# Senryoku/zflac

Hardware: AMD Instinct MI355X
Metric: Msamples/s decoded (bit-exact) + achieved HBM GB/s, 4096-blk stereo (higher is better)
Workload: dtype int32; 1 GPU; C5 shard: 1250 stereo 16-bit mid/side FLAC streams/GPU x 32 frames x 4096 samples, LPC order 8, partition order 4; streams_total=1250, parallelism=stream-shard x1

## Files before the change

### include/zflac_hip.h

```cpp
#ifndef ZFLAC_HIP_H
#define ZFLAC_HIP_H

#include <stddef.h>
#include <stdint.h>

#ifdef __cplusplus
extern "C" {
#endif

#define ZFLAC_OK 0
#define ZFLAC_E_INVALID_SIGNATURE 1
#define ZFLAC_E_INVALID_METADATA_HEADER 2
#define ZFLAC_E_MISSING_STREAMINFO 3
#define ZFLAC_E_UNIMPLEMENTED 4
#define ZFLAC_E_INVALID_CHECKSUM 5
#define ZFLAC_E_INVALID_FRAME_HEADER 6
#define ZFLAC_E_INCONSISTENT_PARAMETERS 7
#define ZFLAC_E_INVALID_CODED_NUMBER 8
#define ZFLAC_E_INVALID_SUBFRAME_HEADER 9
#define ZFLAC_E_INVALID_RESIDUAL_CODING 10
#define ZFLAC_E_END_OF_STREAM 11
#define ZFLAC_E_OUT_OF_MEMORY 12
#define ZFLAC_E_DEVICE 13
#define ZFLAC_E_INVALID_ARGUMENT 14
#define ZFLAC_E_OUT_OF_DOMAIN 15
#define ZFLAC_E_FRAME_CRC 16

#define ZFLAC_S8 0
#define ZFLAC_S16 1
#define ZFLAC_S32 2

typedef struct zflac_info {
    uint8_t channels;
    uint8_t bits_per_sample;
    uint8_t sample_kind;
    uint8_t reserved;
    uint32_t sample_rate;
    uint64_t n_samples;
    uint64_t samples_bytes;
} zflac_info;

typedef struct zflac_stream {
    const uint8_t *data;
    size_t len;
} zflac_stream;

typedef struct zflac_timings {
    double scan_ms;
    double decode_ms;
    double verify_ms;
    double total_ms;
    uint64_t frames;
    uint64_t input_bytes;
    uint64_t output_bytes;
    uint64_t samples;
    double walk_ms;
    double md5_ms;
    double plan_ms;
    double upload_ms;
    double run_wall_ms;
    double read_ms;
    double host_md5_ms;
    double crc16_ms;
    uint32_t rest_launches;
    uint32_t sequential_streams;
} zflac_timings;

typedef struct zflac_batch zflac_batch;

int zflac_hip_open(const uint8_t *buf, size_t len, int device, zflac_batch **out_batch, zflac_info *info);
int zflac_hip_open_ex(const uint8_t *buf, size_t len, int device, int flags, zflac_batch **out_batch,
                      zflac_info *info);
int zflac_hip_read(zflac_batch *b, void *out_samples, size_t out_bytes);
void zflac_hip_close(zflac_batch *b);

int zflac_hip_batch_create(const zflac_stream *streams, size_t n, int device, int flags, zflac_batch **out);
int zflac_hip_batch_run(zflac_batch *b);
int zflac_hip_batch_submit(zflac_batch *b);
int zflac_hip_batch_wait(zflac_batch *b);
int zflac_hip_batch_ready(zflac_batch *b);
int zflac_hip_batch_info(zflac_batch *b, size_t i, zflac_info *info);
int zflac_hip_batch_read(zflac_batch *b, size_t i, void *out, size_t out_bytes, int verify_md5);
int zflac_hip_batch_md5(zflac_batch *b, size_t i, uint8_t *digest16);
const void *zflac_hip_batch_device_samples(zflac_batch *b, size_t i);
int zflac_hip_batch_timings(zflac_batch *b, zflac_timings *t);
int zflac_hip_batch_timings_ex(zflac_batch *b, zflac_timings *t, size_t size);
#define ZFLAC_TIMINGS_V1_SIZE 80
#define ZFLAC_BUCKET_8 1u
#define ZFLAC_BUCKET_4 2u
#define ZFLAC_BUCKET_16 4u
#define ZFLAC_BUCKET_32 8u
#define ZFLAC_BUCKET_MIX_8 16u
#define ZFLAC_BUCKET_MIX_32 32u
#define ZFLAC_BUCKET_12 64u
#define ZFLAC_BUCKET_ALL 127u
int zflac_hip_batch_decode_buckets(zflac_batch *b, uint32_t *used, uint32_t *planned);
size_t zflac_hip_batch_size(zflac_batch *b);
void zflac_hip_batch_destroy(zflac_batch *b);

#define ZFLAC_EXPORT_F32 0
#define ZFLAC_EXPORT_F16 1
#define ZFLAC_EXPORT_BF16 2
#define ZFLAC_EXPORT_I32 3
#define ZFLAC_LAYOUT_PLANAR 0
#define ZFLAC_LAYOUT_INTERLEAVED 1
typedef struct zflac_export_desc {
    uint32_t size;
    uint8_t dtype, layout;
    uint16_t channels;
    uint64_t frames;
    const uint64_t *starts;
} zflac_export_desc;
int zflac_hip_batch_export(zflac_batch *b, const zflac_export_desc *d, void *dst_device, size_t dst_bytes,
                           uint64_t *valid_frames, void *stream);
int zflac_hip_batch_export_ms(zflac_batch *b, double *ms);

typedef struct zflac_resample_desc {
    uint32_t size;
    uint8_t dtype, layout;
    uint16_t channels;
    uint64_t frames;
    const uint64_t *starts;
    uint32_t sample_rate;
    uint16_t zeros;
    uint16_t reserved;
    double rolloff;
    double beta;
} zflac_resample_desc;
int zflac_hip_batch_export_resampled(zflac_batch *b, const zflac_resample_desc *d, void *dst_device,
                                     size_t dst_bytes, uint64_t *valid_frames, void *stream);
uint64_t zflac_hip_resampled_frames(uint64_t n_frames, uint32_t rate_in, uint32_t rate_out);
int zflac_hip_batch_resample_tables(zflac_batch *b, uint64_t *built, uint64_t *held_floats);

#define ZFLAC_FLAG_TIMING 1
#define ZFLAC_FLAG_FORCE_SLOW 2
#define ZFLAC_FLAG_DEVICE_MD5 4
#define ZFLAC_FLAG_CHECK_CRC16 8
#define ZFLAC_FLAG_WALK_LANE 16
#define ZFLAC_FLAG_WALK_WAVE 32

const char *zflac_hip_error_name(int code);
int zflac_hip_device_count(void);
const char *zflac_hip_version(void);
const char *zflac_hip_build_id(void);
#define ZFLAC_HIP_ABI_VERSION 5
int zflac_hip_abi_version(void);

#ifdef __cplusplus
}
#endif
#endif
```

### zflac_amd/_lib.py

```python
from __future__ import annotations

import ctypes
import os

_HERE = os.path.dirname(os.path.abspath(__file__))
lib_path = os.environ.get("ZFLAC_HIP_LIB") or os.path.join(_HERE, "libzflac_hip.so")


class zflac_info(ctypes.Structure):
    _fields_ = [("channels", ctypes.c_uint8), ("bits_per_sample", ctypes.c_uint8),
                ("sample_kind", ctypes.c_uint8), ("reserved", ctypes.c_uint8),
                ("sample_rate", ctypes.c_uint32), ("n_samples", ctypes.c_uint64),
                ("samples_bytes", ctypes.c_uint64)]


class zflac_stream(ctypes.Structure):
    _fields_ = [("data", ctypes.c_void_p), ("len", ctypes.c_size_t)]


class zflac_timings(ctypes.Structure):
    _fields_ = [("scan_ms", ctypes.c_double), ("decode_ms", ctypes.c_double), ("verify_ms", ctypes.c_double),
                ("total_ms", ctypes.c_double), ("frames", ctypes.c_uint64), ("input_bytes", ctypes.c_uint64),
                ("output_bytes", ctypes.c_uint64), ("samples", ctypes.c_uint64), ("walk_ms", ctypes.c_double),
                ("md5_ms", ctypes.c_double), ("plan_ms", ctypes.c_double), ("upload_ms", ctypes.c_double),
                ("run_wall_ms", ctypes.c_double), ("read_ms", ctypes.c_double), ("host_md5_ms", ctypes.c_double),
                ("crc16_ms", ctypes.c_double), ("rest_launches", ctypes.c_uint32), ("sequential_streams", ctypes.c_uint32)]


class zflac_export_desc(ctypes.Structure):
    _fields_ = [("size", ctypes.c_uint32), ("dtype", ctypes.c_uint8), ("layout", ctypes.c_uint8),
                ("channels", ctypes.c_uint16), ("frames", ctypes.c_uint64), ("starts", ctypes.POINTER(ctypes.c_uint64))]


class zflac_resample_desc(ctypes.Structure):
    _fields_ = [("size", ctypes.c_uint32), ("dtype", ctypes.c_uint8), ("layout", ctypes.c_uint8),
                ("channels", ctypes.c_uint16), ("frames", ctypes.c_uint64), ("starts", ctypes.POINTER(ctypes.c_uint64)),
                ("sample_rate", ctypes.c_uint32), ("zeros", ctypes.c_uint16), ("reserved", ctypes.c_uint16),
                ("rolloff", ctypes.c_double), ("beta", ctypes.c_double)]


_P = ctypes.c_void_p
SIGNATURES = {
    "zflac_hip_open": (ctypes.c_int, [ctypes.c_char_p, ctypes.c_size_t, ctypes.c_int, ctypes.POINTER(_P),
                                      ctypes.POINTER(zflac_info)]),
    "zflac_hip_open_ex": (ctypes.c_int, [ctypes.c_char_p, ctypes.c_size_t, ctypes.c_int, ctypes.c_int,
                                         ctypes.POINTER(_P), ctypes.POINTER(zflac_info)]),
    "zflac_hip_read": (ctypes.c_int, [_P, _P, ctypes.c_size_t]),
    "zflac_hip_close": (None, [_P]),
    "zflac_hip_batch_create": (ctypes.c_int, [ctypes.POINTER(zflac_stream), ctypes.c_size_t, ctypes.c_int,
                                              ctypes.c_int, ctypes.POINTER(_P)]),
    "zflac_hip_batch_run": (ctypes.c_int, [_P]),
    "zflac_hip_batch_submit": (ctypes.c_int, [_P]),
    "zflac_hip_batch_wait": (ctypes.c_int, [_P]),
    "zflac_hip_batch_ready": (ctypes.c_int, [_P]),
    "zflac_hip_batch_info": (ctypes.c_int, [_P, ctypes.c_size_t, ctypes.POINTER(zflac_info)]),
    "zflac_hip_batch_read": (ctypes.c_int, [_P, ctypes.c_size_t, _P, ctypes.c_size_t, ctypes.c_int]),
    "zflac_hip_batch_md5": (ctypes.c_int, [_P, ctypes.c_size_t, ctypes.c_char_p]),
    "zflac_hip_batch_device_samples": (_P, [_P, ctypes.c_size_t]),
    "zflac_hip_batch_timings": (ctypes.c_int, [_P, ctypes.POINTER(zflac_timings)]),
    "zflac_hip_batch_timings_ex": (ctypes.c_int, [_P, ctypes.POINTER(zflac_timings), ctypes.c_size_t]),
    "zflac_hip_abi_version": (ctypes.c_int, []),
    "zflac_hip_batch_export": (ctypes.c_int, [_P, ctypes.POINTER(zflac_export_desc), _P, ctypes.c_size_t,
                                              ctypes.POINTER(ctypes.c_uint64), _P]),
    "zflac_hip_batch_export_ms": (ctypes.c_int, [_P, ctypes.POINTER(ctypes.c_double)]),
    "zflac_hip_batch_export_resampled": (ctypes.c_int, [_P, ctypes.POINTER(zflac_resample_desc), _P, ctypes.c_size_t,
                                                        ctypes.POINTER(ctypes.c_uint64), _P]),
    "zflac_hip_resampled_frames": (ctypes.c_uint64, [ctypes.c_uint64, ctypes.c_uint32, ctypes.c_uint32]),
    "zflac_hip_batch_resample_tables": (ctypes.c_int, [_P, ctypes.POINTER(ctypes.c_uint64),
                                                       ctypes.POINTER(ctypes.c_uint64)]),
    "zflac_hip_batch_decode_buckets": (ctypes.c_int, [_P, ctypes.POINTER(ctypes.c_uint32),
                                                      ctypes.POINTER(ctypes.c_uint32)]),
    "zflac_hip_batch_size": (ctypes.c_size_t, [_P]),
    "zflac_hip_batch_destroy": (None, [_P]),
    "zflac_hip_error_name": (ctypes.c_char_p, [ctypes.c_int]),
    "zflac_hip_device_count": (ctypes.c_int, []),
    "zflac_hip_version": (ctypes.c_char_p, []),
    "zflac_hip_build_id": (ctypes.c_char_p, []),
}

FLAG_TIMING = 1
FLAG_FORCE_SLOW = 2
FLAG_DEVICE_MD5 = 4
FLAG_CHECK_CRC16 = 8
FLAG_WALK_LANE = 16
FLAG_WALK_WAVE = 32
EXPORT_F32 = 0
EXPORT_F16 = 1
EXPORT_BF16 = 2
EXPORT_I32 = 3
LAYOUT_PLANAR = 0
LAYOUT_INTERLEAVED = 1
BUCKET_8 = 1
BUCKET_4 = 2
BUCKET_16 = 4
BUCKET_32 = 8
BUCKET_MIX_8 = 16
BUCKET_MIX_32 = 32
BUCKET_12 = 64
BUCKET_ALL = 127

_lib = None


def load():
    global _lib
    if _lib is None:
        if not os.path.exists(lib_path):
            try:
                from . import build as _build

                _build.build()
            except Exception as e:
                raise RuntimeError(f"libzflac_hip.so is missing and could not be built: {e}") from e
        lib = ctypes.CDLL(lib_path)
        for name, (res, args) in SIGNATURES.items():
            fn = getattr(lib, name)
            fn.restype = res
            fn.argtypes = args
        _lib = lib
    return _lib
```

### zflac_amd/api.py

```python
from __future__ import annotations

import ctypes
import dataclasses

import numpy as np

from . import _lib, errors

_DTYPES = {0: np.int8, 1: np.int16, 2: np.int32}
_TAGS = {0: "s8", 1: "s16", 2: "s32"}


@dataclasses.dataclass
class Samples:

    tag: str
    values: np.ndarray

    @property
    def s8(self) -> np.ndarray:
        return self._arm("s8")

    @property
    def s16(self) -> np.ndarray:
        return self._arm("s16")

    @property
    def s32(self) -> np.ndarray:
        return self._arm("s32")

    def _arm(self, tag):
        if self.tag != tag:
            raise AttributeError(f"inactive union field {tag!r} (active: {self.tag!r})")
        return self.values


@dataclasses.dataclass
class DecodedFLAC:

    channels: int
    sample_rate: int
    bits_per_sample: int
    samples: Samples

    def deinit(self, allocator=None) -> None:
        self.samples = Samples(self.samples.tag, self.samples.values[:0])


def _read_all(reader) -> bytes:
    if isinstance(reader, (bytes, bytearray, memoryview)):
        return bytes(reader)
    if hasattr(reader, "read"):
        return reader.read()
    raise TypeError("decode() expects bytes or a reader with .read()")


def device_count() -> int:
    return _lib.load().zflac_hip_device_count()


def build_id() -> str:
    return _lib.load().zflac_hip_build_id().decode()


def _aligned_empty(nbytes: int, dtype) -> np.ndarray:
    raw = np.empty(nbytes + 32, dtype=np.uint8)
    off = (-raw.ctypes.data) % 32
    return raw[off:off + nbytes].view(dtype)


def decode(reader, device: int = 0, timings: dict | None = None, check_crc16: bool = False) -> DecodedFLAC:
    data = _read_all(reader)
    L = _lib.load()
    handle = ctypes.c_void_p()
    info = _lib.zflac_info()
    flags = _lib.FLAG_CHECK_CRC16 if check_crc16 else 0
    rc = L.zflac_hip_open_ex(data, len(data), device, flags, ctypes.byref(handle), ctypes.byref(info))
    try:
        errors.check(rc)
        out = _aligned_empty(info.samples_bytes, _DTYPES[info.sample_kind])
        rc = L.zflac_hip_read(handle, out.ctypes.data_as(ctypes.c_void_p) if info.samples_bytes else None,
                              info.samples_bytes)
        errors.check(rc)
        if timings is not None:
            t = _lib.zflac_timings()
            L.zflac_hip_batch_timings_ex(handle, ctypes.byref(t), ctypes.sizeof(t))
            timings.update({name: getattr(t, name) for name, _ in _lib.zflac_timings._fields_})
        return DecodedFLAC(info.channels, info.sample_rate, info.bits_per_sample,
                           Samples(_TAGS[info.sample_kind], out))
    finally:
        if handle:
            L.zflac_hip_close(handle)


class Batch:

    def __init__(self, streams, device: int = 0, timing: bool = False, force_slow: bool = False,
                 device_md5: bool = False, check_crc16: bool = False, walk: str | None = None):
        self._L = _lib.load()
        self.device = device
        self._bufs = [bytes(s) for s in streams]
        arr = (_lib.zflac_stream * len(self._bufs))()
        self._keep = []
        for i, b in enumerate(self._bufs):
            cb = ctypes.create_string_buffer(b, len(b))
            self._keep.append(cb)
            arr[i].data = ctypes.cast(cb, ctypes.c_void_p)
            arr[i].len = len(b)
        flags = ((_lib.FLAG_TIMING if timing else 0) | (_lib.FLAG_FORCE_SLOW if force_slow else 0)
                 | (_lib.FLAG_DEVICE_MD5 if device_md5 else 0) | (_lib.FLAG_CHECK_CRC16 if check_crc16 else 0)
                 | {None: 0, "lane": _lib.FLAG_WALK_LANE, "wave": _lib.FLAG_WALK_WAVE}[walk])
        self._h = ctypes.c_void_p()
        rc = self._L.zflac_hip_batch_create(arr, len(self._bufs), device, flags, ctypes.byref(self._h))
        self._keep = None
        errors.check(rc, "batch_create")

    def __len__(self):
        return len(self._bufs)

    def run(self) -> None:
        errors.check(self._L.zflac_hip_batch_run(self._h), "batch_run")

    def submit(self) -> None:
        errors.check(self._L.zflac_hip_batch_submit(self._h), "batch_submit")

    def wait(self) -> None:
        errors.check(self._L.zflac_hip_batch_wait(self._h), "batch_wait")

    def ready(self) -> bool:
        rc = self._L.zflac_hip_batch_ready(self._h)
        if rc < 0:
            errors.check(-rc, "batch_ready")
        return rc == 1

    def info(self, i: int):
        inf = _lib.zflac_info()
        rc = self._L.zflac_hip_batch_info(self._h, i, ctypes.byref(inf))
        return rc, inf

    def error_name(self, i: int) -> str:
        return errors.NAMES.get(self.info(i)[0], "Unknown")

    def read(self, i: int, verify_md5: bool = True) -> DecodedFLAC:
        rc, inf = self.info(i)
        errors.check(rc)
        out = _aligned_empty(inf.samples_bytes, _DTYPES[inf.sample_kind])
        rc = self._L.zflac_hip_batch_read(self._h, i, out.ctypes.data_as(ctypes.c_void_p) if inf.samples_bytes
                                          else None, inf.samples_bytes, 1 if verify_md5 else 0)
        errors.check(rc)
        return DecodedFLAC(inf.channels, inf.sample_rate, inf.bits_per_sample, Samples(_TAGS[inf.sample_kind], out))

    def md5(self, i: int):
        buf = ctypes.create_string_buffer(16)
        rc = self._L.zflac_hip_batch_md5(self._h, i, buf)
        return None if rc else buf.raw

    def timings(self):
        t = _lib.zflac_timings()
        rc = self._L.zflac_hip_batch_timings_ex(self._h, ctypes.byref(t), ctypes.sizeof(t))
        return None if rc else t

    def decode_buckets(self):
        used, planned = ctypes.c_uint32(), ctypes.c_uint32()
        errors.check(self._L.zflac_hip_batch_decode_buckets(self._h, ctypes.byref(used), ctypes.byref(planned)),
                     "batch_decode_buckets")
        return used.value, planned.value

    def device_samples(self, i: int) -> int:
        return self._L.zflac_hip_batch_device_samples(self._h, i) or 0

    def close(self):
        if getattr(self, "_h", None):
            self._L.zflac_hip_batch_destroy(self._h)
            self._h = None

    def __del__(self):
        try:
            self.close()
        except Exception:
            pass


def decode_many(streams, device: int = 0, verify_md5: bool = True, device_md5: bool = True):
    b = Batch(streams, device, device_md5=device_md5 and verify_md5)
    try:
        b.run()
        out = []
        for i in range(len(b)):
            try:
                out.append(b.read(i, verify_md5))
            except errors.ZflacError as e:
                out.append(e)
        return out
    finally:
        b.close()
```

### zflac_amd/build.py

```python
from __future__ import annotations

import os
import subprocess
import sys
import time

HERE = os.path.dirname(os.path.abspath(__file__))
ROOT = os.path.dirname(HERE)
CSRC = os.path.join(HERE, "csrc")
LIB = os.path.join(HERE, "libzflac_hip.so")
SOURCES = [os.path.join(CSRC, f"decode_k{k}_{lay}{mix}.hip") for k in (1, 2, 0) for lay in ("stereo", "mono", "multi")
           for mix in ("", "_mix")]
SOURCES += [os.path.join(CSRC, n) for n in ("scan.hip", "md5.hip", "crc16.hip", "walk_wave.hip", "export.hip",
                                            "resample.hip", "stream_plan.cpp", "resample_plan.cpp", "pipeline.cpp",
                                            "seq_planner.cpp", "md5_host.cpp", "abi.cpp")]
HEADERS = [os.path.join(CSRC, n) for n in ("common.h", "frame_header.h", "device_common.h", "launch.h", "stream_plan.h",
                                           "resample_plan.h", "export_tile.h", "batch.h", "md5.hpp", "decode.inc")]
DEPS = SOURCES + HEADERS + [os.path.join(ROOT, "include", "zflac_hip.h")]
ARCH = os.environ.get("ZFLAC_OFFLOAD_ARCH", "gfx950")
CFLAGS = ["-O3", "-std=c++20", "-fPIC", "-Wall", "-Wno-unused-function"]


def source_fingerprint(defines=()) -> str:
    import hashlib

    h = hashlib.sha256(f"{ARCH}|{' '.join(CFLAGS)}|{' '.join(sorted(defines))}".encode())
    for d in sorted(DEPS):
        h.update(os.path.basename(d).encode())
        with open(d, "rb") as f:
            h.update(f.read())
    return h.hexdigest()


def sources_present() -> bool:
    return all(os.path.exists(d) for d in DEPS)


def needs_build() -> bool:
    if not os.path.exists(LIB):
        return True
    t = os.path.getmtime(LIB)
    return any(os.path.getmtime(d) > t for d in DEPS)


def lib_build_id(path: str | None = None) -> str | None:
    import re

    try:
        with open(path or LIB, "rb") as f:
            m = re.search(rb"src=([0-9a-f]{64})", f.read())
    except OSError:
        return None
    return m.group(0).decode() if m else None


def _obj_deps(src: str):
    if src.endswith("abi.cpp"):
        return list(DEPS)
    hdrs = [h for h in HEADERS if not h.endswith("decode.inc") or "decode_k" in src]
    return [src] + hdrs + [os.path.join(ROOT, "include", "zflac_hip.h")]


def build(force: bool = False, verbose: bool = False, defines=(), out: str | None = None, units=None) -> str:
    lib = out or LIB
    if not force and not defines and not out and not needs_build():
        return LIB
    if units:
        build()
        units = set(units) | {"abi.cpp"}
    objs = []
    tag = "_".join(d.replace("=", "-") for d in defines)
    build_dir = os.path.join(HERE, "_build" + ("_" + tag if tag else ""))
    os.makedirs(build_dir, exist_ok=True)
    procs = []
    fp = source_fingerprint(defines)
    jobs = max(1, min(int(os.environ.get("MAX_JOBS", "8")), os.cpu_count() or 1, 16))
    for src in SOURCES:
        if units and os.path.basename(src) not in units:
            objs.append(os.path.join(HERE, "_build", os.path.basename(src) + ".o"))
            continue
        obj = os.path.join(build_dir, os.path.basename(src) + ".o")
        if not force and os.path.exists(obj) and os.path.getmtime(obj) >= max(os.path.getmtime(d)
                                                                               for d in _obj_deps(src)):
            objs.append(obj)
            continue
        cmd = ["hipcc", f"--offload-arch={ARCH}"] + CFLAGS + ["-I", os.path.join(ROOT, "include"), "-c", src, "-o", obj]
        cmd[1:1] = [f"-D{d}" for d in defines]
        if src.endswith(".hip"):
            cmd[1:1] = ["-x", "hip"]
        if src.endswith("_plan.cpp"):
            cmd[1:1] = ["-x", "c++"]
        if src.endswith("abi.cpp"):
            cmd[1:1] = [f'-DZFLAC_BUILD_ID="src={fp}"']
        if verbose:
            print(" ".join(cmd))
        while sum(p.poll() is None for _, p in procs) >= jobs:
            time.sleep(0.2)
        procs.append((src, subprocess.Popen(cmd)))
        objs.append(obj)
    failed = [src for src, p in procs if p.wait() != 0]
    if failed:
        raise RuntimeError(f"hipcc failed for {failed}")
    os.makedirs(os.path.dirname(lib), exist_ok=True)
    cmd = ["hipcc", f"--offload-arch={ARCH}", "-shared", "-fPIC", "-o", lib] + objs
    subprocess.check_call(cmd)
    return lib


if __name__ == "__main__":
    a = sys.argv[1:]
    out = a[a.index("-o") + 1] if "-o" in a else None
    units = a[a.index("--units") + 1].split(",") if "--units" in a else None
    build(force="--force" in a, verbose=True, defines=[x[2:] for x in a if x.startswith("-D")], out=out, units=units)
```

### zflac_amd/csrc/abi.cpp

```cpp
#include <cstring>
#include <new>
#include <vector>

#include "batch.h"
#include "launch.h"

using namespace zflac;

zflac_batch::~zflac_batch() {
    if (exp_pending) (void)hipEventSynchronize(ev_exp);
    if (stream) (void)hipStreamSynchronize(stream);
    if (ev_done) (void)hipEventSynchronize(ev_done);
    if (md5_pending) {
        try {
            hub_release(this);
        } catch (...) {
        }
        try {
            hub_forget(this);
        } catch (...) {
        }
    }
    if (md5_hub && ev_md5) (void)hipEventSynchronize(ev_md5);
    if (front) (void)hipStreamSynchronize(front);
    classes.clear();
    for (auto& s : streams) s.override_out.reset();
    for (auto& e : ev)
        if (e) (void)hipEventDestroy(e);
    if (ev_done) (void)hipEventDestroy(ev_done);
    if (ev_md5) (void)hipEventDestroy(ev_md5);
    if (pipe_pin) (void)hipHostFree(pipe_pin);
    if (exp_pin) (void)hipHostFree(exp_pin);
    if (ev_exp_copy) (void)hipEventDestroy(ev_exp_copy);
    if (ev_exp) (void)hipEventDestroy(ev_exp);
    for (auto& e : ev_exp_t)
        if (e) (void)hipEventDestroy(e);
    if (stream) (void)hipStreamDestroy(stream);
    if (front) (void)hipStreamDestroy(front);
    if (front_join) (void)hipEventDestroy(front_join);
}

namespace {

struct ExportShape {
    size_t n;
    uint64_t T, C, esz, tiles;
    uint32_t vec;
};

bool export_shape(zflac_batch* b, uint32_t size, uint32_t want_size, int dtype, int max_dtype, int layout,
                  uint64_t channels, uint64_t frames, const void* dst, size_t dst_bytes, ExportShape& s) {
    if (!b || !dst || size != want_size) return false;
    if (dtype > max_dtype || layout > ZFLAC_LAYOUT_INTERLEAVED || !channels || !frames) return false;
    if (!b->ran || b->submitted) return false;
    s.n = b->streams.size();
    s.T = frames;
    s.C = channels;
    s.esz = (dtype == ZFLAC_EXPORT_F16 || dtype == ZFLAC_EXPORT_BF16) ? 2 : 4;
    const unsigned __int128 need = (unsigned __int128)s.n * s.C * s.T * s.esz;
    if (need > (unsigned __int128)dst_bytes) return false;
    s.tiles = (s.T + EXPORT_TILE - 1) / EXPORT_TILE;
    if ((unsigned __int128)s.n * s.tiles > 0x7FFFFFFFull) return false;
    const uint64_t row_bytes = (layout == ZFLAC_LAYOUT_PLANAR ? s.T : s.T * s.C) * s.esz;
    s.vec = (reinterpret_cast<uintptr_t>(dst) % 16 == 0 && row_bytes % 16 == 0) ? 1u : 0u;
    return true;
}

ExportRow export_row(const StreamState& s, uint64_t start) {
    ExportRow r;
    std::memset(&r, 0, sizeof(r));
    r.start = start;
    r.kind = s.info.sample_kind;
    if (!s.err && s.info.channels && s.dev_samples) {
        r.nch = s.info.channels;
        r.n_frames = s.info.n_samples / s.info.channels;
        if (r.start < r.n_frames) r.src = s.dev_samples;
    }
    return r;
}

bool export_begin(zflac_batch* b, size_t n, void* stream, hipStream_t st) {
    if (!b->exp_pin) {
        ck(hipHostMalloc(reinterpret_cast<void**>(&b->exp_pin), n * sizeof(ResampleRow), hipHostMallocDefault));
        b->exp_rows.alloc(n * sizeof(ResampleRow));
        ck(hipEventCreateWithFlags(&b->ev_exp_copy, hipEventDisableTiming));
        ck(hipEventCreateWithFlags(&b->ev_exp, hipEventDisableTiming));
    }
    if (b->exp_any) {
        ck(hipEventSynchronize(b->ev_exp_copy));
        ck(hipStreamWaitEvent(st, b->ev_exp, 0));
    }
    const bool timed = !stream && (b->flags & ZFLAC_FLAG_TIMING);
    if (timed)
        for (auto& e : b->ev_exp_t)
            if (!e) ck(hipEventCreate(&e));
    return timed;
}

template <typename Launch>
void export_run(zflac_batch* b, size_t bytes, bool timed, void* stream, hipStream_t st, Launch launch) {
    if (timed) ck(hipEventRecord(b->ev_exp_t[0], st));
    ck(hipMemcpyAsync(b->exp_rows.p, b->exp_pin, bytes, hipMemcpyHostToDevice, st));
    ck(hipEventRecord(b->ev_exp_copy, st));
    const hipError_t le = launch();
    ck(hipEventRecord(b->ev_exp, st));
    b->exp_any = true;
    ck(le);
    if (timed) ck(hipEventRecord(b->ev_exp_t[1], st));
    if (stream) {
        b->exp_pending = true;
    } else {
        ck(hipStreamSynchronize(st));
        if (timed) {
            float ms = 0;
            ck(hipEventElapsedTime(&ms, b->ev_exp_t[0], b->ev_exp_t[1]));
            b->export_ms = ms;
        }
    }
}

ResampleTable* resample_table(zflac_batch* b, uint32_t fin, const zflac_resample_desc* d, const ResampleRatio& ratio) {
    for (auto& t : b->rs_tables)
        if (t->fin == fin && t->fout == d->sample_rate && t->zeros == d->zeros && t->rolloff == d->rolloff &&
            t->beta == d->beta)
            return t.get();
    auto t = std::make_unique<ResampleTable>();
    t->fin = fin;
    t->fout = d->sample_rate;
    t->zeros = d->zeros;
    t->rolloff = d->rolloff;
    t->beta = d->beta;
    t->ratio = ratio;
    std::vector<float> h;
    resample_taps(ratio, d->zeros, d->beta, h);
    t->taps.alloc(h.size());
    ck(hipMemcpy(t->taps.p, h.data(), h.size() * sizeof(float), hipMemcpyHostToDevice));
    b->rs_built++;
    b->rs_tables.push_back(std::move(t));
    return b->rs_tables.back().get();
}

}

extern "C" {

const char* zflac_hip_error_name(int code) {
    switch (code) {
        case 0: return "OK";
        case 1: return "InvalidSignature";
        case 2: return "InvalidMetadataHeader";
        case 3: return "MissingStreaminfo";
        case 4: return "Unimplemented";
        case 5: return "InvalidChecksum";
        case 6: return "InvalidFrameHeader";
        case 7: return "InconsistentParameters";
        case 8: return "InvalidCodedNumber";
        case 9: return "InvalidSubframeHeader";
        case 10: return "InvalidResidualCodingMethod";
        case 11: return "EndOfStream";
        case 12: return "OutOfMemory";
        case 13: return "DeviceError";
        case 14: return "InvalidArgument";
        case 15: return "OutOfDomain";
        case 16: return "FrameCrcMismatch";
        default: return "Unknown";
    }
}

int zflac_hip_device_count(void) {
    int n = 0;
    if (hipGetDeviceCount(&n) != hipSuccess) return 0;
    return n;
}

const char* zflac_hip_version(void) { return "zflac_hip gfx950 r4"; }

#ifndef ZFLAC_BUILD_ID
#define ZFLAC_BUILD_ID "unknown"
#endif
const char* zflac_hip_build_id(void) { return ZFLAC_BUILD_ID; }

int zflac_hip_batch_create(const zflac_stream* streams, size_t n, int device, int flags, zflac_batch** out) {
    return create_batch(streams, n, device, flags, out);
}

static void drain_failed_submit(zflac_batch* b) {
    try {
        hub_forget(b);
    } catch (...) {
    }
    (void)hipStreamSynchronize(b->stream);
    if (b->rs) (void)hipStreamSynchronize(b->rs);
    if (b->front) (void)hipStreamSynchronize(b->front);
    b->rs = b->stream;
    b->submitted = false;
}

int zflac_hip_batch_submit(zflac_batch* b) {
    if (!b || b->submitted) return E_INVALID_ARGUMENT;
    b->ran = false;
    try {
        b->submit_t0 = now_ms();
        b->submitted = true;
        submit_batch(b);
    } catch (const DeviceError&) {
        drain_failed_submit(b);
        return E_DEVICE;
    } catch (const std::bad_alloc&) {
        drain_failed_submit(b);
        return E_OUT_OF_MEMORY;
    } catch (const std::exception&) {
        drain_failed_submit(b);
        return E_DEVICE;
    }
    return E_OK;
}

int zflac_hip_batch_wait(zflac_batch* b) {
    if (!b || !b->submitted) return E_INVALID_ARGUMENT;
    b->submitted = false;
    int rc = E_OK;
    try {
        finish_batch(b);
        b->timings.run_wall_ms = now_ms() - b->submit_t0;
        b->ran = true;
    } catch (const DeviceError&) {
        rc = E_DEVICE;
    } catch (const std::bad_alloc&) {
        rc = E_OUT_OF_MEMORY;
    } catch (const std::exception&) {
        rc = E_DEVICE;
    }
    if (rc != E_OK && b->md5_pending) {
        try {
            hub_forget(b);
        } catch (...) {
        }
    }
    return rc;
}

int zflac_hip_batch_ready(zflac_batch* b) {
    if (!b || !b->submitted) return -E_INVALID_ARGUMENT;
    hipError_t e = hipEventQuery(b->ev_done);
    if (e == hipSuccess && b->md5_hub) {
        try {
            Md5Hub& h = md5_hub(b->device);
            std::lock_guard<std::mutex> lock(h.mu);
            if (b->md5_pending) {
                if (!h.any || hipEventQuery(h.last) == hipSuccess) hub_flush(h);
                return 0;
            }
            if (b->md5_failed) return -E_DEVICE;
        } catch (const DeviceError&) {
            return -E_DEVICE;
        }
        e = hipEventQuery(b->ev_md5);
    }
    if (e == hipSuccess) return 1;
    if (e == hipErrorNotReady) return 0;
    return -E_DEVICE;
}

int zflac_hip_batch_run(zflac_batch* b) {
    const int rc = zflac_hip_batch_submit(b);
    return rc ? rc : zflac_hip_batch_wait(b);
}

size_t zflac_hip_batch_size(zflac_batch* b) { return b ? b->streams.size() : 0; }

int zflac_hip_batch_info(zflac_batch* b, size_t i, zflac_info* info) {
    if (!b || !b->ran || i >= b->streams.size()) return E_INVALID_ARGUMENT;
    const StreamState& s = b->streams[i];
    if (info) *info = s.info;
    return s.err;
}

const void* zflac_hip_batch_device_samples(zflac_batch* b, size_t i) {
    if (!b || !b->ran || i >= b->streams.size() || b->streams[i].err) return nullptr;
    return b->streams[i].dev_samples;
}

int zflac_hip_batch_read(zflac_batch* b, size_t i, void* out, size_t out_bytes, int verify_md5) {
    if (!b || !b->ran || i >= b->streams.size()) return E_INVALID_ARGUMENT;
    StreamState& s = b->streams[i];
    if (s.err) return s.err;
    if (out_bytes < s.info.samples_bytes || (!out && s.info.samples_bytes)) return E_INVALID_ARGUMENT;
    try {
        ck(hipSetDevice(b->device));
        return read_samples(b, s, out, verify_md5 && !s.md5_dev);
    } catch (const DeviceError&) {
        return E_DEVICE;
    } catch (const std::exception&) {
        return E_DEVICE;
    }
}

int zflac_hip_batch_md5(zflac_batch* b, size_t i, uint8_t* digest) {
    if (!b || !b->ran || i >= b->streams.size() || !digest) return E_INVALID_ARGUMENT;
    const StreamState& s = b->streams[i];
    if (!s.md5_dev) return E_INVALID_ARGUMENT;
    std::memcpy(digest, s.md5_dig, 16);
    return E_OK;
}

int zflac_hip_batch_timings(zflac_batch* b, zflac_timings* t) {
    return zflac_hip_batch_timings_ex(b, t, ZFLAC_TIMINGS_V1_SIZE);
}

int zflac_hip_batch_timings_ex(zflac_batch* b, zflac_timings* t, size_t size) {
    if (!b || !t || size == 0) return E_INVALID_ARGUMENT;
    std::memcpy(t, &b->timings, std::min(size, sizeof(zflac_timings)));
    if (size > sizeof(zflac_timings)) std::memset(reinterpret_cast<uint8_t*>(t) + sizeof(zflac_timings), 0,
                                                  size - sizeof(zflac_timings));
    return b->have_timing ? E_OK : E_INVALID_ARGUMENT;
}

int zflac_hip_abi_version(void) { return ZFLAC_HIP_ABI_VERSION; }

int zflac_hip_batch_export(zflac_batch* b, const zflac_export_desc* d, void* dst_device, size_t dst_bytes,
                           uint64_t* valid_frames, void* stream) {
    ExportShape s;
    if (!d || !export_shape(b, d->size, sizeof(zflac_export_desc), d->dtype, ZFLAC_EXPORT_I32, d->layout, d->channels,
                            d->frames, dst_device, dst_bytes, s))
        return E_INVALID_ARGUMENT;
    const size_t n = s.n;
    for (size_t i = 0; valid_frames && i < n; i++) {
        const StreamState& st = b->streams[i];
        const uint64_t start = d->starts ? d->starts[i] : 0;
        const uint64_t nf = (st.err || !st.info.channels) ? 0 : st.info.n_samples / st.info.channels;
        valid_frames[i] = nf > start ? std::min(nf - start, s.T) : 0;
    }
    if (n == 0) return E_OK;
    try {
        DeviceScope scope(b->device);
        hipStream_t st = stream ? static_cast<hipStream_t>(stream) : b->stream;
        const bool timed = export_begin(b, n, stream, st);
        ExportRow* rows = reinterpret_cast<ExportRow*>(b->exp_pin);
        for (size_t i = 0; i < n; i++) rows[i] = export_row(b->streams[i], d->starts ? d->starts[i] : 0);
        ExportArgs a;
        std::memset(&a, 0, sizeof(a));
        a.rows = reinterpret_cast<const ExportRow*>(b->exp_rows.p);
        a.dst = dst_device;
        a.frames = s.T;
        a.channels = (uint32_t)s.C;
        a.n_rows = (uint32_t)n;
        a.tiles = (uint32_t)s.tiles;
        a.vec = s.vec;
        export_run(b, n * sizeof(ExportRow), timed, stream, st,
                   [&] { return launch_export(d->dtype, d->layout, a, st); });
    } catch (const DeviceError&) {
        return E_DEVICE;
    } catch (const std::bad_alloc&) {
        return E_OUT_OF_MEMORY;
    }
    return E_OK;
}

uint64_t zflac_hip_resampled_frames(uint64_t n_frames, uint32_t rate_in, uint32_t rate_out) {
    return resampled_frames(n_frames, rate_in, rate_out);
}

int zflac_hip_batch_export_resampled(zflac_batch* b, const zflac_resample_desc* d, void* dst_device, size_t dst_bytes,
                                     uint64_t* valid_frames, void* stream) {
    ExportShape s;
    if (!d || !export_shape(b, d->size, sizeof(zflac_resample_desc), d->dtype, ZFLAC_EXPORT_BF16, d->layout,
                            d->channels, d->frames, dst_device, dst_bytes, s))
        return E_INVALID_ARGUMENT;
    if (!d->sample_rate || d->sample_rate > RESAMPLE_MAX_RATE || d->reserved ||
        !resample_params_ok(d->zeros, d->rolloff, d->beta))
        return E_INVALID_ARGUMENT;
    const size_t n = s.n;
    struct Need {
        uint32_t fin;
        ResampleRatio ratio;
    };
    std::vector<Need> needs;
    std::vector<int> plan(n, -1);
    std::vector<uint64_t> n_out(n, 0);
    uint64_t floats = 0, tiles = s.tiles;
    try {
        for (size_t i = 0; i < n; i++) {
            const StreamState& st = b->streams[i];
            if (st.err || !st.info.channels || !st.info.sample_rate) continue;
            const uint64_t nf = st.info.n_samples / st.info.channels;
            const uint32_t fin = st.info.sample_rate;
            if (fin == d->sample_rate) {
                n_out[i] = nf;
                continue;
            }
            n_out[i] = resampled_frames(nf, fin, d->sample_rate);
            int k = 0;
            while (k < (int)needs.size() && needs[k].fin != fin) k++;
            if (k == (int)needs.size()) {
                Need nd;
                nd.fin = fin;
                if (!resample_ratio(fin, d->sample_rate, d->zeros, d->rolloff, nd.ratio)) return E_INVALID_ARGUMENT;
                if (nd.ratio.K > RESAMPLE_MAX_TAPS) return E_INVALID_ARGUMENT;
                floats += nd.ratio.table_floats();
                if (floats > RESAMPLE_MAX_TABLE_FLOATS) return E_INVALID_ARGUMENT;
                needs.push_back(nd);
            }
            plan[i] = k;
            const ResampleTile rt = resample_tile(needs[k].ratio, std::min<uint64_t>(st.info.channels, s.C));
            tiles = std::max(tiles, (s.T + rt.tile - 1) / rt.tile);
        }
    } catch (const std::bad_alloc&) {
        return E_OUT_OF_MEMORY;
    }
    if ((unsigned __int128)n * tiles > 0x7FFFFFFFull) return E_INVALID_ARGUMENT;
    for (size_t i = 0; valid_frames && i < n; i++) {
        const uint64_t start = d->starts ? d->starts[i] : 0;
        valid_frames[i] = n_out[i] > start ? std::min(n_out[i] - start, s.T) : 0;
    }
    if (n == 0) return E_OK;
    try {
        DeviceScope scope(b->device);
        hipStream_t st = stream ? static_cast<hipStream_t>(stream) : b->stream;
        uint64_t held = 0;
        for (auto& t : b->rs_tables) held += t->ratio.table_floats();
        if (held + floats > RESAMPLE_MAX_TABLE_FLOATS) {
            std::erase_if(b->rs_tables, [&](const std::unique_ptr<ResampleTable>& t) {
                if (t->fout == d->sample_rate && t->zeros == d->zeros && t->rolloff == d->rolloff && t->beta == d->beta)
                    for (const Need& nd : needs)
                        if (nd.fin == t->fin) return false;
                return true;
            });
        }
        std::vector<const ResampleTable*> tabs;
        for (const Need& nd : needs) tabs.push_back(resample_table(b, nd.fin, d, nd.ratio));
        const bool timed = export_begin(b, n, stream, st);
        ResampleRow* rows = reinterpret_cast<ResampleRow*>(b->exp_pin);
        for (size_t i = 0; i < n; i++) {
            const StreamState& ss = b->streams[i];
            ResampleRow r;
            std::memset(&r, 0, sizeof(r));
            const uint64_t start = d->starts ? d->starts[i] : 0;
            if (plan[i] < 0) {
                r.e = export_row(ss, start);
                if (!n_out[i]) r.e.src = nullptr;
            } else {
                const ResampleTable* t = tabs[plan[i]];
                const ResampleTile rt = resample_tile(t->ratio, std::min<uint64_t>(ss.info.channels, s.C));
                r.e = export_row(ss, 0);
                r.e.start = start;
                r.n_out = n_out[i];
                if (r.e.src && start < r.n_out) {
                    r.taps = t->taps.p;
                    r.L = t->ratio.L;
                    r.M = t->ratio.M;
                    r.W = t->ratio.W;
                    r.K = (uint32_t)t->ratio.K;
                    r.tile = rt.tile;
                    r.cg = rt.cg;
                    r.tab_lds = rt.tab_lds;
                } else {
                    r.e.src = nullptr;
                }
            }
            rows[i] = r;
        }
        ResampleArgs a;
        std::memset(&a, 0, sizeof(a));
        a.rows = reinterpret_cast<const ResampleRow*>(b->exp_rows.p);
        a.dst = dst_device;
        a.frames = s.T;
        a.channels = (uint32_t)s.C;
        a.n_rows = (uint32_t)n;
        a.tiles = (uint32_t)tiles;
        a.vec = s.vec;
        export_run(b, n * sizeof(ResampleRow), timed, stream, st,
                   [&] { return launch_resample(d->dtype, d->layout, a, st); });
    } catch (const DeviceError&) {
        return E_DEVICE;
    } catch (const std::bad_alloc&) {
        return E_OUT_OF_MEMORY;
    }
    return E_OK;
}

int zflac_hip_batch_resample_tables(zflac_batch* b, uint64_t* built, uint64_t* held_floats) {
    if (!b) return E_INVALID_ARGUMENT;
    if (built) *built = b->rs_built;
    if (held_floats) {
        *held_floats = 0;
        for (auto& t : b->rs_tables) *held_floats += t->ratio.table_floats();
    }
    return E_OK;
}

static_assert(ZFLAC_BUCKET_8 == bucket_bit(8, false) && ZFLAC_BUCKET_4 == bucket_bit(4, false) &&
                  ZFLAC_BUCKET_16 == bucket_bit(16, false) && ZFLAC_BUCKET_32 == bucket_bit(32, false) &&
                  ZFLAC_BUCKET_MIX_8 == bucket_bit(8, true) && ZFLAC_BUCKET_MIX_32 == bucket_bit(32, true) &&
                  ZFLAC_BUCKET_12 == bucket_bit(12, false) && ZFLAC_BUCKET_ALL == BUCKET_MASK_ALL,
              "ZFLAC_BUCKET_* (zflac_hip.h) and bucket_bit() (common.h) disagree");

int zflac_hip_batch_decode_buckets(zflac_batch* b, uint32_t* used, uint32_t* planned) {
    if (!b || !used || !planned || !b->ran || b->submitted) return E_INVALID_ARGUMENT;
    *used = b->buckets_used;
    *planned = b->buckets_planned;
    return E_OK;
}

int zflac_hip_batch_export_ms(zflac_batch* b, double* ms) {
    if (!b || !ms || b->export_ms < 0) return E_INVALID_ARGUMENT;
    *ms = b->export_ms;
    return E_OK;
}

#ifdef ZFLAC_PROBE
extern "C" int zflac_hip_probe(zflac_batch* b, unsigned long long* out, int n) {
    if (!b || b->classes.empty() || n > (int)(PROBE_BYTES / 8)) return E_INVALID_ARGUMENT;
    auto& C = *b->classes[0];
    uint8_t* p = reinterpret_cast<uint8_t*>(C.dummy.p) + DUMMY_BYTES;
    if (hipMemcpy(out, p, n * 8, hipMemcpyDeviceToHost) != hipSuccess) return E_DEVICE;
    if (hipMemset(p, 0, PROBE_BYTES) != hipSuccess) return E_DEVICE;
    return E_OK;
}
#endif

#ifdef ZFLAC_REPLAY
extern "C" int zflac_hip_replay(zflac_batch** bs, int nb, int reps, int what, double* ms) {
    try {
        if (nb <= 0 || !bs || !ms) return E_INVALID_ARGUMENT;
        ck(hipSetDevice(bs[0]->device));
        for (int i = 0; i < nb; i++) {
            ck(hipStreamSynchronize(bs[i]->rs));
            bs[i]->rs = next_run_stream(bs[i]->device);
        }
        const double t0 = now_ms();
        for (int r = 0; r < reps; r++) {
            for (int i = 0; i < nb; i++) {
                zflac_batch* b = bs[i];
                Class& C = *b->classes[0];
                if (what == 4) {
                    enqueue_class(b, C, false, false);
                    continue;
                }
                if (what >= 8) {
                    const ScanArgs sa = scan_args(C);
                    ck(launch_scan(sa, b->rs));
                    if (what == 16) {
                        ck(launch_scan_chunks(C.chunk_cnt.p, C.chunk_units.p, sa.n_chunks, C.chunk_off.p,
                                              C.chunk_uoff.p, C.misc.p, b->rs));
                        ck(launch_compact(compact_args(C), b->rs));
                    }
                    continue;
                }
                DecodeArgs da = decode_args(C);
                da.full_mask = C.full_mask;
                const uint32_t mf = std::min(C.grid_frames, C.cap);
                if (what & 1) ck(launch_walk_k1(da, mf, b->rs));
                if (what & 2) ck(launch_decode_k1_stereo(da, mf, b->rs));
            }
        }
        for (int i = 0; i < nb; i++) ck(hipStreamSynchronize(bs[i]->rs));
        *ms = now_ms() - t0;
        for (int i = 0; i < nb; i++) bs[i]->rs = bs[i]->stream;
        return E_OK;
    } catch (const DeviceError&) {
        return E_DEVICE;
    }
}
#endif

void zflac_hip_batch_destroy(zflac_batch* b) {
    if (!b) return;
    (void)hipSetDevice(b->device);
    delete b;
}

int zflac_hip_open(const uint8_t* buf, size_t len, int device, zflac_batch** out_batch, zflac_info* info) {
    return zflac_hip_open_ex(buf, len, device, 0, out_batch, info);
}

int zflac_hip_open_ex(const uint8_t* buf, size_t len, int device, int flags, zflac_batch** out_batch,
                      zflac_info* info) {
    if (!out_batch) return E_INVALID_ARGUMENT;
    zflac_stream s{buf, len};
    int rc = create_batch(&s, 1, device, flags, out_batch);
    if (rc) return rc;
    rc = zflac_hip_batch_run(*out_batch);
    if (rc) return rc;
    return zflac_hip_batch_info(*out_batch, 0, info);
}

int zflac_hip_read(zflac_batch* b, void* out_samples, size_t out_bytes) {
    return zflac_hip_batch_read(b, 0, out_samples, out_bytes, 1);
}

void zflac_hip_close(zflac_batch* b) { zflac_hip_batch_destroy(b); }

}
```

### zflac_amd/csrc/batch.h

```cpp
#pragma once
#include <hip/hip_runtime.h>

#include <algorithm>
#include <atomic>
#include <chrono>
#include <cstdint>
#include <memory>
#include <mutex>
#include <vector>

#include "../../include/zflac_hip.h"
#include "common.h"
#include "resample_plan.h"
#include "stream_plan.h"

namespace zflac {

inline double now_ms() {
    return std::chrono::duration<double, std::milli>(std::chrono::steady_clock::now().time_since_epoch()).count();
}

struct DeviceError {};
inline void ck(hipError_t e) {
    if (e != hipSuccess) throw DeviceError{};
}

template <typename T>
struct DevBuf {
    T* p = nullptr;
    size_t n = 0;
    DevBuf() = default;
    DevBuf(const DevBuf&) = delete;
    DevBuf& operator=(const DevBuf&) = delete;
    ~DevBuf() { release(); }
    void release() {
        if (p) (void)hipFree(p);
        p = nullptr;
        n = 0;
    }
    void alloc(size_t count) {
        if (count <= n && p) return;
        release();
        ck(hipMalloc(reinterpret_cast<void**>(&p), std::max<size_t>(count, 1) * sizeof(T)));
        n = count;
    }
};

struct ResampleTable {
    uint32_t fin = 0, fout = 0, zeros = 0;
    double rolloff = 0, beta = 0;
    ResampleRatio ratio;
    DevBuf<float> taps;
};

struct StreamState : StreamPlan {
    int cls = -1;
    uint32_t slot = 0;
    int err = 0;
    zflac_info info = {};
    const void* dev_samples = nullptr;
    int md5_dev = 0;
    uint8_t md5_dig[16] = {};
    std::unique_ptr<DevBuf<uint8_t>> override_out;
};

struct Class {
    int kind = 1;
    int nch = 2;
    std::vector<uint32_t> members;
    std::vector<StreamDesc> desc;
    std::vector<ChunkDesc> chunks;
    uint64_t in_bytes = 0, out_elems = 0;
    uint32_t cap = 0;
    uint64_t est_frames = 0;
    uint32_t grid_frames = 0;
    uint32_t full_mask = 0;
    bool redone = false;
    DevBuf<uint8_t> in;
    DevBuf<uint8_t> out;
    DevBuf<StreamDesc> d_desc;
    DevBuf<ChunkDesc> d_chunks;
    DevBuf<uint32_t> chunk_cnt, chunk_off, chunk_slot_units, misc;
    uint32_t* status = nullptr;
    DevBuf<unsigned long long> chunk_units, chunk_uoff;
    DevBuf<uint64_t> chunk_slots;
    DevBuf<uint64_t> c_pos, c_out, c_end;
    DevBuf<uint32_t> c_stream, c_info, c_rate, sub, group_mb;
    DevBuf<int32_t> c_err;
    DevBuf<uint32_t> crc_bad;
    DevBuf<uint8_t> dummy;
    struct Pinned {
        uint32_t* p = nullptr;
        ~Pinned() {
            if (p) (void)hipHostFree(p);
        }
    } pin;
    uint32_t* h_misc = nullptr;
    uint32_t* h_status = nullptr;
    bool any_unknown = false;
    DevBuf<uint64_t> units;
    uint64_t* h_units = nullptr;
};

struct DeviceScope {
    int prev = -1;
    explicit DeviceScope(int dev) {
        if (hipGetDevice(&prev) != hipSuccess) prev = -1;
        if (prev != dev) ck(hipSetDevice(dev));
    }
    ~DeviceScope() {
        int cur = -1;
        if (prev >= 0 && hipGetDevice(&cur) == hipSuccess && cur != prev) (void)hipSetDevice(prev);
    }
};

struct Uploader {
    static constexpr uint64_t WIN = 32ull << 20;
    std::mutex mu;
    uint8_t* pin[2] = {nullptr, nullptr};
    hipEvent_t done[2] = {nullptr, nullptr};
    bool used[2] = {false, false};
};

constexpr int MAX_HUB_STREAMS = 4;
struct Md5Hub {
    std::mutex mu;
    hipStream_t st[MAX_HUB_STREAMS] = {};
    uint32_t n_st = 1, next = 0;
    hipEvent_t last = nullptr;
    bool any = false;
    std::vector<zflac_batch*> pend;
    uint32_t runs = 8;
    int device = 0;
};

constexpr int MAX_RUN_STREAMS = 8;
struct DeviceStreams {
    std::mutex mu;
    hipStream_t run[MAX_RUN_STREAMS] = {};
    uint32_t n_run = 3, next = 0;
    Md5Hub hub;
    DeviceStreams();
};

DeviceStreams& device_streams(int device);
Md5Hub& md5_hub(int device);
hipStream_t next_run_stream(int device);
void hub_flush(Md5Hub& h);
void hub_release(zflac_batch* b);
void hub_forget(zflac_batch* b);
int read_samples(zflac_batch* b, StreamState& s, void* out, bool hash);
void plan_md5_pipeline(zflac_batch* b);
void finish_md5(zflac_batch* b, bool timing);

DecodeArgs decode_args(Class& C);
ScanArgs scan_args(Class& C);
CompactArgs compact_args(Class& C);
hipError_t launch_decode(int kind, const DecodeArgs& a, uint32_t max_frames, hipStream_t st,
                         hipEvent_t mid = nullptr, hipStream_t front = nullptr, hipEvent_t join = nullptr,
                         uint64_t est_frames = 0, int flags = 0);
void enqueue_class(zflac_batch* b, Class& C, bool timing_first, bool timing_last);
void submit_batch(zflac_batch* b);
void finish_batch(zflac_batch* b);
int create_batch(const zflac_stream* streams, size_t n, int device, int flags, zflac_batch** out);

void finish_stream_sequential(zflac_batch* b, Class& C, uint32_t slot, const std::vector<uint32_t>& h_chunk_off,
                              uint32_t nframes);

}

struct zflac_batch {
    int device = 0;
    int flags = 0;
    hipStream_t stream = nullptr;
    hipStream_t front = nullptr;
    hipEvent_t front_join = nullptr;
    std::vector<zflac::StreamState> streams;
    std::vector<std::unique_ptr<zflac::Class>> classes;
    hipEvent_t ev[10] = {};
    hipEvent_t ev_done = nullptr;
    hipStream_t rs = nullptr;
    hipEvent_t ev_md5 = nullptr;
    std::atomic<bool> md5_pending{false};
    bool md5_failed = false;
    bool md5_hub = false;
    bool have_timing = false;
    bool ran = false;
    bool submitted = false;
    double submit_t0 = 0;
    zflac::DevBuf<zflac::Md5Job> md5_jobs;
    zflac::DevBuf<uint32_t> md5_dig;
    zflac::DevBuf<zflac::Md5Job> pipe_jobs;
    int pipe_coop = -1;
    zflac::DevBuf<uint32_t> pipe_dig;
    std::vector<uint32_t> pipe_who;
    uint32_t* pipe_pin = nullptr;
    zflac_timings timings = {};
    uint8_t* exp_pin = nullptr;
    zflac::DevBuf<uint8_t> exp_rows;
    hipEvent_t ev_exp_copy = nullptr, ev_exp = nullptr;
    hipEvent_t ev_exp_t[2] = {};
    bool exp_any = false;
    bool exp_pending = false;
    double export_ms = -1;
    std::vector<std::unique_ptr<zflac::ResampleTable>> rs_tables;
    uint64_t rs_built = 0;
    uint32_t buckets_used = 0, buckets_planned = 0;
    ~zflac_batch();
};
```

### zflac_amd/csrc/common.h

```cpp
#pragma once
#include <cstdint>

#ifdef __HIPCC__
#define ZFLAC_HD __host__ __device__
#else
#define ZFLAC_HD
#endif

namespace zflac {

enum Err : int {
    E_OK = 0,
    E_INVALID_SIGNATURE = 1,
    E_INVALID_METADATA_HEADER = 2,
    E_MISSING_STREAMINFO = 3,
    E_UNIMPLEMENTED = 4,
    E_INVALID_CHECKSUM = 5,
    E_INVALID_FRAME_HEADER = 6,
    E_INCONSISTENT_PARAMETERS = 7,
    E_INVALID_CODED_NUMBER = 8,
    E_INVALID_SUBFRAME_HEADER = 9,
    E_INVALID_RESIDUAL_CODING = 10,
    E_END_OF_STREAM = 11,
    E_OUT_OF_MEMORY = 12,
    E_DEVICE = 13,
    E_INVALID_ARGUMENT = 14,
    E_OUT_OF_DOMAIN = 15,
    E_FRAME_CRC = 16,
};

struct StreamDesc {
    uint64_t in_begin;
    uint64_t in_end;
    uint64_t out_base;
    uint64_t out_cap;
    uint64_t total;
    uint32_t rate_hz;
    uint32_t si_rate;
    uint32_t first_chunk;
    uint32_t end_chunk;
    uint8_t byte1;
    uint8_t nch;
    uint8_t dcode;
    uint8_t si_bps;
    uint8_t valid_total;
    uint8_t justify;
    uint8_t pad_[2];
};

struct ChunkDesc {
    uint64_t begin;
    uint64_t end;
    uint32_t stream;
    uint32_t pad_;
};

constexpr uint32_t INFO_PRE_ERR = 1u << 28;
constexpr uint32_t INFO_CRC_EOF = 1u << 29;

constexpr int SCAN_THREADS = 256;
#ifndef ZFLAC_SCAN_BPT
#define ZFLAC_SCAN_BPT 128
#endif
constexpr int SCAN_BYTES_PER_THREAD = ZFLAC_SCAN_BPT;
constexpr uint64_t CHUNK_BYTES = (uint64_t)SCAN_THREADS * SCAN_BYTES_PER_THREAD;
constexpr int CHUNK_CAP = 64;
constexpr uint64_t INPUT_PAD = 4096;
constexpr int MAX_CH = 8;
#ifndef ZFLAC_WAVE_WALK_MAX_FRAMES
#define ZFLAC_WAVE_WALK_MAX_FRAMES 16384
#endif
constexpr uint64_t WAVE_WALK_MAX_FRAMES = ZFLAC_WAVE_WALK_MAX_FRAMES;
constexpr uint64_t DUMMY_BYTES = 64 * 64 * 32;
constexpr uint64_t PROBE_BYTES = 256;

struct ScanArgs {
    const uint8_t* in;
    const StreamDesc* streams;
    const ChunkDesc* chunks;
    uint32_t n_chunks;
    uint32_t* chunk_cnt;
    unsigned long long* chunk_units;
    uint64_t* chunk_slots;
    uint32_t* chunk_slot_units;
    uint32_t* status;
    uint32_t n_status;
    uint32_t* misc;
};

struct CompactArgs {
    const uint8_t* in;
    const StreamDesc* streams;
    const ChunkDesc* chunks;
    uint32_t n_chunks;
    const uint32_t* chunk_cnt;
    const uint64_t* chunk_slots;
    const uint32_t* chunk_slot_units;
    const uint32_t* chunk_off;
    const unsigned long long* chunk_uoff;
    uint32_t cap;
    uint64_t* c_pos;
    uint32_t* c_stream;
    uint64_t* c_out;
    uint32_t* overflow;
};

struct DecodeArgs {
    const uint8_t* in;
    uint64_t in_size;
    void* out;
    const StreamDesc* streams;
    const uint64_t* c_pos;
    const uint32_t* c_stream;
    const uint64_t* c_out;
    const uint32_t* n_frames;
    uint32_t n_frames_host;
    uint32_t cap;
    uint64_t* c_end;
    int32_t* c_err;
    uint32_t* c_info;
    uint32_t* c_rate;
    int nch;
    int write;
    void* dummy;
    uint32_t* sub_start;
    uint32_t* group_mb;
    uint32_t* bucket_used;
    uint32_t full_mask;
    uint32_t rest;
    uint32_t rest_only;
};

constexpr uint32_t SPARSE_DECODE_BLOCKS = 256;

ZFLAC_HD inline constexpr uint32_t bucket_bit(uint32_t mb, bool mix) {
    return mix ? (mb <= 8 ? 16u : 32u)
               : (mb == 8 ? 1u : (mb == 4 ? 2u : (mb == 16 ? 4u : (mb == 12 ? 64u : 8u))));
}
constexpr uint32_t BUCKET_MASK_ALL = 127u;

enum Md5Mode : uint32_t {
    MD5_RAW = 0,
    MD5_S16_SHIFT = 1,
    MD5_S32_SHIFT = 2,
    MD5_S24 = 3,
};

struct Md5Job {
    const uint8_t* data;
    uint64_t n;
    uint32_t mode;
    uint32_t js;
    uint32_t width;
    uint32_t pad_;
    const uint32_t* status;
};

constexpr int MD5_MAX_SEGS = 16;
struct Md5Segs {
    const Md5Job* jobs[MD5_MAX_SEGS];
    uint32_t* dig[MD5_MAX_SEGS];
    uint32_t start[MD5_MAX_SEGS + 1];
    uint32_t nseg;
};

struct VerifyArgs {
    const StreamDesc* streams;
    uint32_t n_streams;
    const uint32_t* chunk_off;
    const uint64_t* c_pos;
    const uint32_t* c_stream;
    const uint64_t* c_out;
    const uint32_t* n_frames;
    uint32_t cap;
    const uint64_t* c_end;
    const int32_t* c_err;
    const uint32_t* c_info;
    const uint32_t* c_rate;
    uint32_t* status;
    uint64_t* units;
};

struct SyncListArgs {
    const uint8_t* in;
    uint64_t lo, hi;
    uint64_t in_end;
    uint32_t si_rate;
    uint32_t rate_hz;
    uint32_t nch, dcode;
    uint64_t* pos;
    uint32_t* count;
    uint32_t cap;
};

struct Crc16Args {
    const uint8_t* in;
    uint64_t in_size;
    const uint64_t* pos;
    const uint64_t* end;
    const int32_t* err;
    const StreamDesc* streams;
    const uint32_t* c_stream;
    const uint64_t* c_out;
    const uint32_t* n_frames;
    uint32_t n_frames_host;
    uint32_t cap;
    uint32_t* bad;
};

struct ExportRow {
    const void* src;
    uint64_t n_frames;
    uint64_t start;
    uint8_t nch;
    uint8_t kind;
    uint8_t pad_[6];
};
static_assert(sizeof(ExportRow) == 32, "ExportRow is the 32-byte record host and kernel share");

constexpr uint32_t EXPORT_THREADS = 256;
constexpr uint32_t EXPORT_GROUP = 16;
constexpr uint64_t EXPORT_TILE = (uint64_t)EXPORT_THREADS * EXPORT_GROUP;

struct ExportArgs {
    const ExportRow* rows;
    void* dst;
    uint64_t frames;
    uint32_t channels;
    uint32_t n_rows;
    uint32_t tiles;
    uint32_t vec;
};

struct ResampleRow {
    ExportRow e;
    const float* taps;
    uint64_t n_out;
    uint32_t L, M;
    uint32_t W, K;
    uint32_t tile;
    uint8_t cg;
    uint8_t tab_lds;
    uint8_t pad_[2];
};
static_assert(sizeof(ResampleRow) == 72, "ResampleRow is the 72-byte record host and kernel share");

constexpr uint32_t RESAMPLE_THREADS = 512;
constexpr uint32_t RESAMPLE_LDS_FLOATS = 20480;
constexpr uint32_t RESAMPLE_LDS_TABLE = 16896;
constexpr uint32_t RESAMPLE_MAX_TILE = 2048;
constexpr uint32_t RESAMPLE_MAX_CG = 4;

struct ResampleArgs {
    const ResampleRow* rows;
    void* dst;
    uint64_t frames;
    uint32_t channels;
    uint32_t n_rows;
    uint32_t tiles;
    uint32_t vec;
};

}
```

### zflac_amd/csrc/device_common.h

```cpp
#pragma once
#include <hip/hip_runtime.h>

#include <atomic>
#include <cstdint>
#include <utility>

#include "common.h"
#include "frame_header.h"

namespace zflac {

__device__ __forceinline__ uint32_t bswap32(uint32_t x) { return __builtin_bswap32(x); }

static __constant__ Crc8Table CRC8 = make_crc8_table();

__device__ __forceinline__ FrameHdr parse_frame_header(const uint8_t* p, uint64_t avail, uint32_t si_rate) {
    return parse_frame_header_t<1>([p](uint32_t i) -> uint32_t { return p[i]; }, avail, si_rate, CRC8.t);
}
__device__ __forceinline__ FrameHdr parse_frame_fields(const uint8_t* p, uint64_t avail, uint32_t si_rate) {
    return parse_frame_header_t<0>([p](uint32_t i) -> uint32_t { return p[i]; }, avail, si_rate, nullptr);
}

__device__ __forceinline__ bool candidate_ok(const FrameHdr& h, const StreamDesc& S) {
    return h.err == 0 && !h.crc_eof && h.crc_ok && h.zero_bit == 0 && h.byte1 == S.byte1 &&
           channels_count(h.chan_code) == S.nch && h.dcode == S.dcode && h.rate == S.rate_hz;
}

}
```

### zflac_amd/csrc/frame_header.h

```cpp
#pragma once
#include <cstdint>

#include "common.h"

#define ZFLAC_HDI ZFLAC_HD inline __attribute__((always_inline))
#ifdef __clang__
#define ZFLAC_UNROLL _Pragma("unroll")
#else
#define ZFLAC_UNROLL _Pragma("GCC unroll 8")
#endif

namespace zflac {

ZFLAC_HDI int channels_count(uint32_t code) {
    return code <= 7 ? (int)code + 1 : (code <= 10 ? 2 : 0);
}
ZFLAC_HDI uint32_t rate_table(uint32_t code) {
    switch (code) {
        case 1: return 88200;
        case 2: return 176400;
        case 3: return 192000;
        case 4: return 8000;
        case 5: return 16000;
        case 6: return 22050;
        case 7: return 24000;
        case 8: return 32000;
        case 9: return 44100;
        case 10: return 48000;
        default: return 96000;
    }
}
ZFLAC_HDI int depth_bits(uint32_t dcode, int si_bps) {
    switch (dcode) {
        case 0: return si_bps;
        case 1: return 8;
        case 2: return 12;
        case 4: return 16;
        case 5: return 20;
        case 6: return 24;
        case 7: return 32;
        default: return -1;
    }
}

struct Crc8Table {
    uint8_t t[256];
};
constexpr Crc8Table make_crc8_table() {
    Crc8Table r{};
    for (int i = 0; i < 256; i++) {
        uint32_t c = (uint32_t)i;
        for (int k = 0; k < 8; k++) c = (c & 0x80) ? ((c << 1) ^ 0x07) & 0xFF : (c << 1) & 0xFF;
        r.t[i] = (uint8_t)c;
    }
    return r;
}

constexpr uint32_t crc8_reduce(uint32_t a) {
    for (int i = 0; i < 4; i++) {
        const uint32_t t = a >> 8;
        a = (t ^ (t << 1) ^ (t << 2)) ^ (a & 0xFFu);
    }
    return a;
}
constexpr uint32_t crc8_3(uint32_t crc, uint32_t w) { return crc8_reduce((w ^ (crc << 16)) << 8); }
constexpr uint32_t crc8_1(uint32_t crc, uint32_t b) { return crc8_reduce((crc ^ b) << 8); }
constexpr bool crc8_fold_matches_table() {
    const Crc8Table t = make_crc8_table();
    for (uint32_t i = 0; i < 256; i++)
        if (crc8_1(0, i) != t.t[i]) return false;
    uint32_t a = 0, b = 0, x = 12345;
    for (int k = 0; k < 300; k++) {
        uint32_t w = 0;
        for (int j = 0; j < 3; j++) {
            x = x * 1103515245u + 12345u;
            const uint32_t by = (x >> 16) & 0xFFu;
            a = t.t[a ^ by];
            w = (w << 8) | by;
        }
        b = crc8_3(b, w);
        if (a != b) return false;
    }
    return true;
}
static_assert(crc8_fold_matches_table(), "register CRC-8 = table CRC-8");

struct FrameHdr {
    uint32_t bs, rate, hdr_len;
    uint32_t chan_code, dcode, byte1, zero_bit, bs_code;
    int err;
    bool crc_eof;
    bool crc_ok;
};

template <int CRC, typename At>
ZFLAC_HDI FrameHdr parse_frame_header_t(At&& at, uint64_t avail, uint32_t si_rate, const uint8_t* crc_tab) {
    FrameHdr h;
    h.bs = h.rate = h.hdr_len = 0;
    h.chan_code = h.dcode = h.byte1 = h.zero_bit = h.bs_code = 0;
    h.err = 0;
    h.crc_eof = false;
    h.crc_ok = false;
    if (avail < 4) { h.err = E_END_OF_STREAM; return h; }
    const uint32_t b0 = at(0), b1 = at(1), b2 = at(2), b3 = at(3);
    h.byte1 = b1;
    h.chan_code = b3 >> 4;
    h.dcode = (b3 >> 1) & 7;
    h.zero_bit = b3 & 1;
    h.bs_code = b2 >> 4;
    if (((b0 << 7) | (b1 >> 1)) != 0x7FFC) { h.err = E_INVALID_FRAME_HEADER; return h; }
    uint32_t idx = 4;
    if (avail <= idx) { h.err = E_END_OF_STREAM; return h; }
    const uint32_t first = at(idx++);
#ifdef __HIP_DEVICE_COMPILE__
    const uint32_t ones = __clz((~first & 0xFFu) << 24) > 8 ? 8 : __clz((~first & 0xFFu) << 24);
#else
    uint32_t ones = 0;
    while (ones < 8 && (first & (0x80u >> ones))) ones++;
#endif
    if (first == 0xFF || ones == 1) { h.err = E_INVALID_CODED_NUMBER; return h; }
    if (ones >= 2) {
        if (avail < (uint64_t)idx + (ones - 1)) { h.err = E_END_OF_STREAM; return h; }
        idx += ones - 1;
    }
    const uint32_t bc = b2 >> 4;
    if (bc == 0) { h.err = E_INVALID_FRAME_HEADER; return h; }
    if (bc == 6) {
        if (avail <= idx) { h.err = E_END_OF_STREAM; return h; }
        h.bs = (uint32_t)at(idx++) + 1;
    } else if (bc == 7) {
        if (avail < (uint64_t)idx + 2) { h.err = E_END_OF_STREAM; return h; }
        const uint32_t v = ((uint32_t)at(idx) << 8) | at(idx + 1);
        idx += 2;
        if (v == 0xFFFF) { h.err = E_INVALID_FRAME_HEADER; return h; }
        h.bs = v + 1;
    } else if (bc == 1) {
        h.bs = 192;
    } else if (bc <= 5) {
        h.bs = 144u << bc;
    } else {
        h.bs = 1u << bc;
    }
    const uint32_t rc = b2 & 15;
    if (rc == 0) {
        h.rate = si_rate;
    } else if (rc == 12) {
        if (avail <= idx) { h.err = E_END_OF_STREAM; return h; }
        h.rate = at(idx++);
    } else if (rc == 13 || rc == 14) {
        if (avail < (uint64_t)idx + 2) { h.err = E_END_OF_STREAM; return h; }
        h.rate = ((uint32_t)at(idx) << 8) | at(idx + 1);
        if (rc == 14) h.rate *= 10;
        idx += 2;
    } else if (rc == 15) {
        h.err = E_INVALID_FRAME_HEADER;
        return h;
    } else {
        h.rate = rate_table(rc);
    }
    h.hdr_len = idx + 1;
    if (avail <= idx) {
        h.crc_eof = true;
        return h;
    }
    if constexpr (CRC == 1) {
        uint32_t crc = 0;
        for (uint32_t i = 0; i < idx; i++) crc = crc_tab[crc ^ at(i)];
        h.crc_ok = crc == at(idx);
    } else if constexpr (CRC == 2) {
        uint32_t crc = 0, i = 0;
        ZFLAC_UNROLL
        for (int g = 0; g < 5; g++) {
            if (i + 3 <= idx) {
                crc = crc8_3(crc, (at(i) << 16) | (at(i + 1) << 8) | at(i + 2));
                i += 3;
            }
        }
        ZFLAC_UNROLL
        for (int g = 0; g < 2; g++) {
            if (i < idx) {
                crc = crc8_1(crc, at(i));
                i++;
            }
        }
        h.crc_ok = crc == at(idx);
    }
    return h;
}

}
```

### zflac_amd/csrc/launch.h

```cpp
#pragma once
#include <hip/hip_runtime.h>

#include <cstdint>

#include "common.h"

namespace zflac {

hipError_t launch_scan(const ScanArgs& a, hipStream_t st);
hipError_t launch_scan_chunks(const uint32_t* cnt, const unsigned long long* units, uint32_t n, uint32_t* off,
                              unsigned long long* uoff, uint32_t* n_frames, hipStream_t st);
hipError_t launch_compact(const CompactArgs& a, hipStream_t st);
hipError_t launch_sync_list(const SyncListArgs& a, hipStream_t st);
hipError_t launch_verify(const VerifyArgs& a, uint32_t max_items, hipStream_t st);

using DecodeLaunch = hipError_t(const DecodeArgs& a, uint32_t max_frames, hipStream_t st);
DecodeLaunch launch_decode_k0_stereo, launch_decode_k0_mono, launch_decode_k0_multi;
DecodeLaunch launch_decode_k1_stereo, launch_decode_k1_mono, launch_decode_k1_multi;
DecodeLaunch launch_decode_k2_stereo, launch_decode_k2_mono, launch_decode_k2_multi;
DecodeLaunch launch_decode_k0_stereo_mix, launch_decode_k0_mono_mix, launch_decode_k0_multi_mix;
DecodeLaunch launch_decode_k1_stereo_mix, launch_decode_k1_mono_mix, launch_decode_k1_multi_mix;
DecodeLaunch launch_decode_k2_stereo_mix, launch_decode_k2_mono_mix, launch_decode_k2_multi_mix;
DecodeLaunch launch_walk_k0, launch_walk_k1, launch_walk_k2;

hipError_t launch_walk_wave(int kind, const DecodeArgs& a, uint32_t max_frames, hipStream_t st);

hipError_t launch_crc16(const Crc16Args& a, uint32_t max_frames, hipStream_t st);

hipError_t launch_md5(const Md5Job* jobs, uint32_t n_jobs, uint32_t* digests, hipStream_t st, int coop_mode);
hipError_t launch_md5_multi(const Md5Segs& sg, hipStream_t st, int coop_mode);

hipError_t launch_export(int dtype, int layout, const ExportArgs& a, hipStream_t st);

hipError_t launch_resample(int dtype, int layout, const ResampleArgs& a, hipStream_t st);

}
```

### zflac_amd/csrc/pipeline.cpp

```cpp
#include <cstdlib>
#include <cstring>
#include <functional>
#include <new>
#include <thread>
#include <unordered_map>

#include "batch.h"
#include "launch.h"

namespace zflac {
namespace {

Uploader& uploader(int device) {
    static std::mutex mu;
    static std::unordered_map<int, Uploader*> per_device;
    std::lock_guard<std::mutex> lock(mu);
    Uploader*& u = per_device[device];
    if (!u) u = new Uploader();
    return *u;
}

void fill_window(uint8_t* dst, uint64_t a, uint64_t b, const std::vector<uint64_t>& in_off,
                 const std::vector<const uint8_t*>& srcs, const std::vector<uint64_t>& lens) {
    size_t m = std::upper_bound(in_off.begin(), in_off.end(), a) - in_off.begin();
    m = m ? m - 1 : 0;
    uint64_t p = a;
    for (; p < b && m < in_off.size(); m++) {
        const uint64_t s0 = in_off[m], s1 = in_off[m] + lens[m];
        if (s1 <= p) continue;
        if (s0 >= b) break;
        if (s0 > p) {
            std::memset(dst + (p - a), 0, s0 - p);
            p = s0;
        }
        const uint64_t e = std::min(s1, b);
        std::memcpy(dst + (p - a), srcs[m] + (p - s0), e - p);
        p = e;
    }
    if (p < b) std::memset(dst + (p - a), 0, b - p);
}

void upload_streams(int device, uint8_t* dev, uint64_t total, const std::vector<uint64_t>& in_off,
                    const std::vector<const uint8_t*>& srcs, const std::vector<uint64_t>& lens, hipStream_t st) {
    Uploader& U = uploader(device);
    std::lock_guard<std::mutex> lock(U.mu);
    for (int k = 0; k < 2; k++) {
        if (!U.pin[k]) ck(hipHostMalloc(reinterpret_cast<void**>(&U.pin[k]), Uploader::WIN, hipHostMallocDefault));
        if (!U.done[k]) ck(hipEventCreate(&U.done[k]));
    }
    int k = 0;
    for (uint64_t a = 0; a < total; a += Uploader::WIN, k ^= 1) {
        const uint64_t b = std::min(a + Uploader::WIN, total);
        if (U.used[k]) ck(hipEventSynchronize(U.done[k]));
        const uint64_t n = b - a;
        const int nt = n >= (8ull << 20) ? 4 : 1;
        std::vector<std::thread> ts;
        for (int t = 1; t < nt; t++)
            ts.emplace_back(fill_window, U.pin[k] + n * t / nt, a + n * t / nt, a + n * (t + 1) / nt,
                            std::cref(in_off), std::cref(srcs), std::cref(lens));
        fill_window(U.pin[k], a, a + n / nt, in_off, srcs, lens);
        for (auto& t : ts) t.join();
        ck(hipMemcpyAsync(dev + a, U.pin[k], n, hipMemcpyHostToDevice, st));
        ck(hipEventRecord(U.done[k], st));
        U.used[k] = true;
    }
    ck(hipStreamSynchronize(st));
}

uint32_t plan_buckets(const zflac_batch* b, const Class& C, const zflac_stream* src) {
    uint32_t mask = bucket_bit(8, false);
    for (uint32_t i : C.members) {
        const StreamState& s = b->streams[i];
        const uint64_t p = s.frames_begin + s.first.hdr_len;
        if (s.first.crc_eof || p >= s.len) continue;
        const uint32_t t = (src[i].data[p] >> 1) & 63;
        const uint32_t ord = t >= 32 ? t - 31 : (t >= 8 && t <= 12 ? t - 8 : 0);
        if (t <= 1) mask |= bucket_bit(8, true) | bucket_bit(32, true);
        else mask |= bucket_bit(ord <= 4 ? 4 : ord <= 8 ? 8 : ord <= 12 ? 12 : ord <= 16 ? 16 : 32, false);
    }
    return mask;
}

constexpr uint64_t UNKNOWN_MAX_PER_BYTE = 4096;

void prescan_unknown_totals(zflac_batch* b, Class& C, std::vector<uint64_t>& units, std::vector<uint64_t>& cands) {
    hipStream_t st = b->stream;
    ck(launch_scan(scan_args(C), st));
    std::vector<uint32_t> cnt(C.chunks.size());
    std::vector<unsigned long long> u(C.chunks.size());
    if (!C.chunks.empty()) {
        ck(hipMemcpyAsync(cnt.data(), C.chunk_cnt.p, cnt.size() * sizeof(uint32_t), hipMemcpyDeviceToHost, st));
        ck(hipMemcpyAsync(u.data(), C.chunk_units.p, u.size() * sizeof(unsigned long long), hipMemcpyDeviceToHost, st));
    }
    ck(hipStreamSynchronize(st));
    units.assign(C.members.size(), 0);
    cands.assign(C.members.size(), 0);
    for (size_t k = 0; k < C.chunks.size(); k++) {
        units[C.chunks[k].stream] += u[k];
        cands[C.chunks[k].stream] += cnt[k];
    }
}

void alloc_class(zflac_batch* b, Class& C, const zflac_stream* src) {
    C.full_mask = plan_buckets(b, C, src);
    const int esz = esz_of_kind(C.kind);
    std::vector<uint64_t> in_off(C.members.size());
    uint64_t off = 0;
    for (size_t m = 0; m < C.members.size(); m++) {
        in_off[m] = off;
        off += (b->streams[C.members[m]].len + 15) & ~(uint64_t)15;
    }
    C.in_bytes = off;
    C.in.alloc(off + INPUT_PAD);
    uint64_t est_frames = 0, grid_frames = 0;
    C.desc.resize(C.members.size());
    C.chunks.clear();
    C.any_unknown = false;
    for (size_t m = 0; m < C.members.size(); m++) {
        StreamState& s = b->streams[C.members[m]];
        s.slot = (uint32_t)m;
        StreamDesc& D = C.desc[m];
        std::memset(&D, 0, sizeof(D));
        D.in_begin = in_off[m] + s.frames_begin;
        D.in_end = in_off[m] + s.len;
        D.valid_total = s.si.total > 0;
        D.total = D.valid_total ? s.si.total * (uint64_t)s.nch : 0;
        D.out_cap = D.total;
        if (!D.valid_total) C.any_unknown = true;
        D.rate_hz = s.first.rate;
        D.si_rate = s.si.sample_rate;
        D.byte1 = (uint8_t)s.first.byte1;
        D.nch = (uint8_t)s.nch;
        D.dcode = (uint8_t)s.first.dcode;
        D.si_bps = (uint8_t)s.si.bps;
        D.justify = justify_of(s.si.bps);
        D.first_chunk = (uint32_t)C.chunks.size();
        const uint64_t abase0 = D.in_begin & ~(uint64_t)15;
        for (uint64_t a = abase0; a < D.in_end; a += CHUNK_BYTES) {
            ChunkDesc ch;
            ch.begin = std::max(a, D.in_begin);
            ch.end = std::min(a + CHUNK_BYTES, D.in_end);
            ch.stream = (uint32_t)m;
            ch.pad_ = 0;
            C.chunks.push_back(ch);
        }
        D.end_chunk = (uint32_t)C.chunks.size();
        const uint64_t minb = std::max<uint64_t>(16, s.si.min_block ? s.si.min_block : 16);
        const uint64_t est = std::min<uint64_t>(s.si.total ? s.si.total / minb : s.len / 16, s.len / 2) + 2;
        if (D.valid_total) est_frames += est;
        const bool fixed = s.si.min_block == s.si.max_block && s.si.min_block >= 16;
        if (D.valid_total) grid_frames += fixed ? (s.si.total + s.si.min_block - 1) / s.si.min_block : est;
    }
    std::vector<const uint8_t*> srcs(C.members.size());
    std::vector<uint64_t> lens(C.members.size());
    for (size_t m = 0; m < C.members.size(); m++) {
        srcs[m] = src[C.members[m]].data;
        lens[m] = b->streams[C.members[m]].len;
    }
    upload_streams(b->device, C.in.p, C.in.n, in_off, srcs, lens, b->stream);
    C.d_desc.alloc(C.desc.size());
    const size_t nc = std::max<size_t>(C.chunks.size(), 1);
    C.d_chunks.alloc(nc);
    if (!C.chunks.empty())
        ck(hipMemcpy(C.d_chunks.p, C.chunks.data(), C.chunks.size() * sizeof(ChunkDesc), hipMemcpyHostToDevice));
    C.chunk_cnt.alloc(nc);
    C.chunk_units.alloc(nc);
    C.chunk_slots.alloc(nc * CHUNK_CAP);
    C.chunk_slot_units.alloc(nc * CHUNK_CAP);
    C.chunk_off.alloc(nc + 1);
    C.chunk_uoff.alloc(nc + 1);
    C.misc.alloc(4 + C.members.size());
    C.status = C.misc.p + 4;
    C.dummy.alloc(DUMMY_BYTES + PROBE_BYTES);
    if (C.any_unknown) {
        ck(hipMemcpy(C.d_desc.p, C.desc.data(), C.desc.size() * sizeof(StreamDesc), hipMemcpyHostToDevice));
        std::vector<uint64_t> units, cands;
        prescan_unknown_totals(b, C, units, cands);
        for (size_t m = 0; m < C.members.size(); m++) {
            StreamDesc& D = C.desc[m];
            if (D.valid_total) continue;
            const uint64_t avail = D.in_end - D.in_begin;
            D.out_cap = units[m] <= UNKNOWN_MAX_PER_BYTE * avail + (1u << 20) ? units[m] : 0;
            est_frames += cands[m] + 2;
            grid_frames += cands[m] + 2;
        }
    }
    const uint64_t align_elems = 32 / (uint64_t)esz;
    auto layout = [&]() {
        uint64_t o = 0;
        for (StreamDesc& D : C.desc) {
            o = (o + align_elems - 1) & ~(align_elems - 1);
            D.out_base = o;
            o += D.out_cap;
        }
        return o;
    };
    uint64_t out = layout();
    if (C.any_unknown) {
        size_t free_b = 0, total_b = 0;
        if (hipMemGetInfo(&free_b, &total_b) != hipSuccess) free_b = 0;
        while (out * esz > free_b / 2) {
            StreamDesc* big = nullptr;
            for (StreamDesc& D : C.desc)
                if (!D.valid_total && D.out_cap && (!big || D.out_cap > big->out_cap)) big = &D;
            if (!big) break;
            big->out_cap = 0;
            out = layout();
        }
    }
    try {
        C.out.alloc(out * esz + 32);
    } catch (const DeviceError&) {
        bool dropped = false;
        for (StreamDesc& D : C.desc)
            if (!D.valid_total && D.out_cap) {
                D.out_cap = 0;
                dropped = true;
            }
        if (!dropped) throw;
        (void)hipGetLastError();
        out = layout();
        C.out.alloc(out * esz + 32);
    }
    C.out_elems = out;
    ck(hipMemcpy(C.d_desc.p, C.desc.data(), C.desc.size() * sizeof(StreamDesc), hipMemcpyHostToDevice));
    const size_t units_at = (4 + C.members.size() + 1) & ~(size_t)1;
    const size_t pin_words = units_at + (C.any_unknown ? 2 * C.members.size() : 0);
    ck(hipHostMalloc(reinterpret_cast<void**>(&C.pin.p), pin_words * sizeof(uint32_t), hipHostMallocDefault));
    std::memset(C.pin.p, 0, pin_words * sizeof(uint32_t));
    C.h_misc = C.pin.p;
    C.h_status = C.pin.p + 4;
    if (C.any_unknown) {
        C.units.alloc(C.members.size());
        C.h_units = reinterpret_cast<uint64_t*>(C.pin.p + units_at);
    }
    C.cap = (uint32_t)std::min<uint64_t>(est_frames + C.chunks.size() * 2 + 1024, 0x7FFFFFFFull);
    C.est_frames = est_frames;
    C.grid_frames = (uint32_t)std::min<uint64_t>(grid_frames + grid_frames / 64 + 64, C.cap);
}

void alloc_candidates(Class& C) {
    C.c_pos.alloc(C.cap);
    C.c_out.alloc(C.cap);
    C.c_end.alloc(C.cap);
    C.c_stream.alloc(C.cap);
    C.c_info.alloc(C.cap);
    C.c_rate.alloc(C.cap);
    C.c_err.alloc(C.cap);
    C.sub.alloc((size_t)C.cap * MAX_CH);
    C.group_mb.alloc((size_t)C.cap / 4 + 2);
}

}

ScanArgs scan_args(Class& C) {
    ScanArgs a;
    std::memset(&a, 0, sizeof(a));
    a.in = C.in.p;
    a.streams = C.d_desc.p;
    a.chunks = C.d_chunks.p;
    a.n_chunks = (uint32_t)C.chunks.size();
    a.chunk_cnt = C.chunk_cnt.p;
    a.chunk_units = C.chunk_units.p;
    a.chunk_slots = C.chunk_slots.p;
    a.chunk_slot_units = C.chunk_slot_units.p;
    a.status = C.status;
    a.n_status = (uint32_t)C.members.size();
    a.misc = C.misc.p;
    return a;
}

CompactArgs compact_args(Class& C) {
    CompactArgs a;
    std::memset(&a, 0, sizeof(a));
    a.in = C.in.p;
    a.streams = C.d_desc.p;
    a.chunks = C.d_chunks.p;
    a.n_chunks = (uint32_t)C.chunks.size();
    a.chunk_cnt = C.chunk_cnt.p;
    a.chunk_slots = C.chunk_slots.p;
    a.chunk_slot_units = C.chunk_slot_units.p;
    a.chunk_off = C.chunk_off.p;
    a.chunk_uoff = C.chunk_uoff.p;
    a.cap = C.cap;
    a.c_pos = C.c_pos.p;
    a.c_stream = C.c_stream.p;
    a.c_out = C.c_out.p;
    a.overflow = C.misc.p + 1;
    return a;
}

static VerifyArgs verify_args(Class& C) {
    VerifyArgs a;
    std::memset(&a, 0, sizeof(a));
    a.streams = C.d_desc.p;
    a.n_streams = (uint32_t)C.members.size();
    a.chunk_off = C.chunk_off.p;
    a.c_pos = C.c_pos.p;
    a.c_stream = C.c_stream.p;
    a.c_out = C.c_out.p;
    a.n_frames = C.misc.p;
    a.cap = C.cap;
    a.c_end = C.c_end.p;
    a.c_err = C.c_err.p;
    a.c_info = C.c_info.p;
    a.c_rate = C.c_rate.p;
    a.status = C.status;
    a.units = C.any_unknown ? C.units.p : nullptr;
    return a;
}

static Crc16Args crc16_args(Class& C) {
    Crc16Args a;
    std::memset(&a, 0, sizeof(a));
    a.in = C.in.p;
    a.in_size = C.in.n;
    a.pos = C.c_pos.p;
    a.end = C.c_end.p;
    a.err = C.c_err.p;
    a.streams = C.d_desc.p;
    a.c_stream = C.c_stream.p;
    a.c_out = C.c_out.p;
    a.n_frames = C.misc.p;
    a.cap = C.cap;
    a.bad = C.crc_bad.p;
    return a;
}

DecodeArgs decode_args(Class& C) {
    DecodeArgs a;
    std::memset(&a, 0, sizeof(a));
    a.in = C.in.p;
    a.in_size = C.in.n;
    a.out = C.out.p;
    a.streams = C.d_desc.p;
    a.c_pos = C.c_pos.p;
    a.c_stream = C.c_stream.p;
    a.c_out = C.c_out.p;
    a.n_frames = C.misc.p;
    a.cap = C.cap;
    a.c_end = C.c_end.p;
    a.c_err = C.c_err.p;
    a.c_info = C.c_info.p;
    a.c_rate = C.c_rate.p;
    a.nch = C.nch;
    a.write = 1;
    a.dummy = C.dummy.p;
    a.sub_start = C.sub.p;
    a.group_mb = C.group_mb.p;
    return a;
}

static bool use_wave_walk(uint64_t frames, int nch, int flags) {
    static const int forced = [] {
        const char* e = std::getenv("ZFLAC_WALK");
        return !e ? 0 : (e[0] == 'w' ? 1 : (e[0] == 'l' ? 2 : 0));
    }();
    if (flags & ZFLAC_FLAG_WALK_WAVE) return true;
    if (flags & ZFLAC_FLAG_WALK_LANE) return false;
    if (forced) return forced == 1;
    return frames * (uint64_t)(nch - 1) < WAVE_WALK_MAX_FRAMES;
}

static constexpr DecodeLaunch* launch_decode_fn[3][3] = {
    {launch_decode_k0_multi, launch_decode_k0_mono, launch_decode_k0_stereo},
    {launch_decode_k1_multi, launch_decode_k1_mono, launch_decode_k1_stereo},
    {launch_decode_k2_multi, launch_decode_k2_mono, launch_decode_k2_stereo},
};
static constexpr DecodeLaunch* launch_walk_fn[3] = {launch_walk_k0, launch_walk_k1, launch_walk_k2};

hipError_t launch_decode(int kind, const DecodeArgs& a, uint32_t max_frames, hipStream_t st, hipEvent_t mid,
                         hipStream_t front, hipEvent_t join, uint64_t est_frames, int flags) {
    const int lay = a.nch == 2 ? 2 : (a.nch == 1 ? 1 : 0);
    hipStream_t ws = front ? front : st;
    if (a.nch > 1 && !a.rest_only) {
        const hipError_t e = use_wave_walk(est_frames ? est_frames : max_frames, a.nch, flags)
                                 ? launch_walk_wave(kind, a, max_frames, ws)
                                 : launch_walk_fn[kind](a, max_frames, ws);
        if (e != hipSuccess) return e;
    }
    if (mid) {
        const hipError_t e = hipEventRecord(mid, ws);
        if (e != hipSuccess) return e;
    }
    if (front) {
        hipError_t e = hipEventRecord(join, front);
        if (e == hipSuccess) e = hipStreamWaitEvent(st, join, 0);
        if (e != hipSuccess) return e;
    }
    return launch_decode_fn[kind][lay](a, max_frames, st);
}

void enqueue_class(zflac_batch* b, Class& C, bool timing_first, bool timing_last) {
    hipStream_t st = b->front ? b->front : b->rs;
    const uint32_t nch = (uint32_t)C.chunks.size();
    if (nch == 0)
        ck(hipMemsetAsync(C.misc.p, 0, (4 + C.members.size()) * sizeof(uint32_t), st));
    if (timing_first) ck(hipEventRecord(b->ev[0], st));
    ck(launch_scan(scan_args(C), st));
    if (nch) ck(launch_scan_chunks(C.chunk_cnt.p, C.chunk_units.p, nch, C.chunk_off.p, C.chunk_uoff.p, C.misc.p, st));
    ck(launch_compact(compact_args(C), st));
    if (timing_last) ck(hipEventRecord(b->ev[1], st));
    DecodeArgs da = decode_args(C);
    da.bucket_used = C.misc.p + 2;
    da.full_mask = C.full_mask;
    ck(launch_decode(C.kind, da, std::min(C.grid_frames, C.cap), b->rs, timing_last ? b->ev[4] : nullptr,
                     b->front, b->front_join, C.est_frames, b->flags));
    st = b->rs;
    if (timing_last) ck(hipEventRecord(b->ev[2], st));
    ck(launch_verify(verify_args(C), C.cap, st));
    if (timing_last) ck(hipEventRecord(b->ev[3], st));
    ck(hipMemcpyAsync(C.h_misc, C.misc.p, (4 + C.members.size()) * sizeof(uint32_t), hipMemcpyDeviceToHost, st));
    if (C.any_unknown)
        ck(hipMemcpyAsync(C.h_units, C.units.p, C.members.size() * sizeof(uint64_t), hipMemcpyDeviceToHost, st));
}

static void enqueue_rest(zflac_batch* b, Class& C) {
    hipStream_t st = b->stream;
    DecodeArgs da = decode_args(C);
    da.full_mask = C.full_mask;
    da.rest_only = 1;
    ck(launch_decode(C.kind, da, std::min(C.grid_frames, C.cap), st));
    ck(hipMemsetAsync(C.status, 0, C.members.size() * sizeof(uint32_t), st));
    ck(launch_verify(verify_args(C), C.cap, st));
    ck(hipMemcpyAsync(C.h_status, C.status, C.members.size() * sizeof(uint32_t), hipMemcpyDeviceToHost, st));
    if (C.any_unknown)
        ck(hipMemcpyAsync(C.h_units, C.units.p, C.members.size() * sizeof(uint64_t), hipMemcpyDeviceToHost, st));
    ck(hipStreamSynchronize(st));
}

void submit_batch(zflac_batch* b) {
    ck(hipSetDevice(b->device));
    const bool timing = (b->flags & ZFLAC_FLAG_TIMING) != 0;
    b->rs = next_run_stream(b->device);
    if (b->exp_pending) {
        ck(hipStreamWaitEvent(b->rs, b->ev_exp, 0));
        if (b->front) ck(hipStreamWaitEvent(b->front, b->ev_exp, 0));
        b->exp_pending = false;
    }
    for (size_t ci = 0; ci < b->classes.size(); ci++) {
        Class& C = *b->classes[ci];
        C.redone = false;
        alloc_candidates(C);
        enqueue_class(b, C, timing && ci == 0, timing && ci + 1 == b->classes.size());
    }
    b->md5_hub = !b->pipe_who.empty() && !std::getenv("ZFLAC_MD5_NOHUB");
    if (!b->pipe_who.empty() && !b->md5_hub) {
        const uint32_t n = (uint32_t)b->pipe_who.size();
        if (timing) ck(hipEventRecord(b->ev[8], b->rs));
        ck(launch_md5(b->pipe_jobs.p, n, b->pipe_dig.p, b->rs, b->pipe_coop));
        if (timing) ck(hipEventRecord(b->ev[9], b->rs));
        ck(hipMemcpyAsync(b->pipe_pin, b->pipe_dig.p, (size_t)n * 16, hipMemcpyDeviceToHost, b->rs));
    }
    ck(hipEventRecord(b->ev_done, b->rs));
    if (b->md5_hub) {
        Md5Hub& h = md5_hub(b->device);
        std::lock_guard<std::mutex> lock(h.mu);
        b->md5_failed = false;
        b->md5_pending = true;
        h.pend.push_back(b);
        if (h.pend.size() >= std::min<uint32_t>(h.runs, MD5_MAX_SEGS)) hub_flush(h);
    }
}

void finish_batch(zflac_batch* b) {
    ck(hipSetDevice(b->device));
    const bool timing = (b->flags & ZFLAC_FLAG_TIMING) != 0;
    ck(hipEventSynchronize(b->ev_done));
    b->rs = b->stream;
    if (b->md5_hub) {
        hub_release(b);
        if (b->md5_failed) {
            b->md5_failed = false;
            throw DeviceError{};
        }
        ck(hipEventSynchronize(b->ev_md5));
    }
    uint32_t rest_launches = 0, sequential = 0, used = 0, planned = 0;
    for (size_t ci = 0; ci < b->classes.size(); ci++) {
        Class& C = *b->classes[ci];
        planned |= C.full_mask;
        for (int attempt = 0; attempt < 3; attempt++) {
            if (!C.h_misc[1] && C.h_misc[0] <= C.cap) break;
            C.cap = std::max<uint32_t>(C.h_misc[0] + 1024, C.cap * 2);
            C.grid_frames = std::max(C.grid_frames, C.h_misc[0]);
            alloc_candidates(C);
            C.redone = true;
            enqueue_class(b, C, false, false);
            ck(hipStreamSynchronize(b->stream));
        }
        if (C.h_misc[0] > C.grid_frames) C.grid_frames = std::min(C.cap, C.h_misc[0] + C.h_misc[0] / 64 + 64);
        used |= C.h_misc[2] & BUCKET_MASK_ALL;
        if (C.full_mask && (C.h_misc[2] & ~C.full_mask)) {
            enqueue_rest(b, C);
            C.redone = true;
            rest_launches++;
            C.full_mask |= C.h_misc[2] & BUCKET_MASK_ALL;
        }
    }
    const bool crc = (b->flags & ZFLAC_FLAG_CHECK_CRC16) != 0;
    b->timings.crc16_ms = 0;
    if (crc && !b->classes.empty()) {
        if (timing) ck(hipEventRecord(b->ev[5], b->stream));
        for (auto& cp : b->classes) {
            Class& C = *cp;
            C.crc_bad.alloc(C.cap);
            ck(launch_crc16(crc16_args(C), std::min(C.h_misc[0], C.cap), b->stream));
        }
        if (timing) ck(hipEventRecord(b->ev[6], b->stream));
        ck(hipStreamSynchronize(b->stream));
        if (timing) {
            float tc = 0;
            ck(hipEventElapsedTime(&tc, b->ev[5], b->ev[6]));
            b->timings.crc16_ms = tc;
        }
    }
    if (timing && !b->classes.empty()) {
        float t01 = 0, t14 = 0, t42 = 0, t23 = 0, t03 = 0;
        ck(hipEventElapsedTime(&t01, b->ev[0], b->ev[1]));
        ck(hipEventElapsedTime(&t14, b->ev[1], b->ev[4]));
        ck(hipEventElapsedTime(&t42, b->ev[4], b->ev[2]));
        ck(hipEventElapsedTime(&t23, b->ev[2], b->ev[3]));
        ck(hipEventElapsedTime(&t03, b->ev[0], b->ev[3]));
        b->timings.scan_ms = t01;
        b->timings.walk_ms = t14;
        b->timings.decode_ms = t42;
        b->timings.verify_ms = t23;
        b->timings.total_ms = t03;
        b->have_timing = true;
    }
    uint64_t frames = 0, in_bytes = 0, out_bytes = 0, samples = 0;
    for (auto& cp : b->classes) {
        Class& C = *cp;
        const int esz = esz_of_kind(C.kind);
        std::vector<uint32_t> h_off, h_crc;
        const uint32_t nfr = std::min(C.h_misc[0], C.cap);
        if (crc && nfr) {
            h_crc.resize(nfr);
            ck(hipMemcpy(h_crc.data(), C.crc_bad.p, nfr * 4, hipMemcpyDeviceToHost));
        }
        for (size_t m = 0; m < C.members.size(); m++) {
            StreamState& s = b->streams[C.members[m]];
            s.override_out.reset();
            s.info = zflac_info{};
            s.info.sample_kind = (uint8_t)C.kind;
            if (C.h_status[m] == 0 && !(b->flags & ZFLAC_FLAG_FORCE_SLOW)) {
                const StreamDesc& D = C.desc[m];
                s.err = 0;
                s.dev_samples = C.out.p + D.out_base * esz;
                s.info.n_samples = D.valid_total ? D.total : C.h_units[m];
                s.info.channels = (uint8_t)s.nch;
                s.info.sample_rate = s.first.rate;
                s.info.bits_per_sample = (uint8_t)depth_bits(s.first.dcode, (int)s.si.bps);
                if (crc) {
                    if (h_off.empty()) {
                        h_off.resize(C.chunks.size() + 1);
                        ck(hipMemcpy(h_off.data(), C.chunk_off.p, h_off.size() * 4, hipMemcpyDeviceToHost));
                    }
                    const uint32_t f0 = std::min(h_off[D.first_chunk], nfr), f1 = std::min(h_off[D.end_chunk], nfr);
                    for (uint32_t f = f0; f < f1; f++)
                        if (h_crc[f]) {
                            s.err = E_FRAME_CRC;
                            s.info = zflac_info{};
                            s.info.sample_kind = (uint8_t)C.kind;
                            break;
                        }
                }
            } else {
                if (h_off.empty()) {
                    h_off.resize(C.chunks.size() + 1);
                    ck(hipMemcpy(h_off.data(), C.chunk_off.p, h_off.size() * 4, hipMemcpyDeviceToHost));
                }
                finish_stream_sequential(b, C, (uint32_t)m, h_off, std::min(C.h_misc[0], C.cap));
                sequential++;
            }
            s.info.samples_bytes = s.info.n_samples * esz;
            if (!s.err) {
                in_bytes += s.len - s.frames_begin;
                out_bytes += s.info.samples_bytes;
                samples += s.info.n_samples;
            }
        }
        frames += std::min(C.h_misc[0], C.cap);
    }
    b->timings.md5_ms = 0;
    if (b->flags & ZFLAC_FLAG_DEVICE_MD5) finish_md5(b, timing && !b->classes.empty());
    else
        for (auto& s : b->streams) s.md5_dev = 0;
    b->timings.frames = frames;
    b->timings.input_bytes = in_bytes;
    b->timings.output_bytes = out_bytes;
    b->timings.samples = samples;
    b->timings.rest_launches = rest_launches;
    b->timings.sequential_streams = sequential;
    b->buckets_used = used;
    b->buckets_planned = planned;
}

int create_batch(const zflac_stream* streams, size_t n, int device, int flags, zflac_batch** out) {
    if (!out || (n && !streams)) return E_INVALID_ARGUMENT;
    *out = nullptr;
    int ndev = 0;
    if (hipGetDeviceCount(&ndev) != hipSuccess || ndev <= 0 || device < 0 || device >= ndev) return E_DEVICE;
    std::unique_ptr<zflac_batch> b(new (std::nothrow) zflac_batch());
    if (!b) return E_OUT_OF_MEMORY;
    b->device = device;
    b->flags = flags;
    try {
        ck(hipSetDevice(device));
        (void)device_streams(device);
        ck(hipStreamCreateWithFlags(&b->stream, hipStreamNonBlocking));
        b->rs = b->stream;
        if (const char* fp = std::getenv("ZFLAC_FRONT_PRIORITY"); fp && fp[0] == '1') {
            int least = 0, greatest = 0;
            ck(hipDeviceGetStreamPriorityRange(&least, &greatest));
            ck(hipStreamCreateWithPriority(&b->front, hipStreamNonBlocking, greatest));
            ck(hipEventCreateWithFlags(&b->front_join, hipEventDisableTiming));
        }
        for (auto& e : b->ev) ck(hipEventCreateWithFlags(&e, hipEventDisableSystemFence));
        ck(hipEventCreateWithFlags(&b->ev_done, hipEventDisableTiming));
        ck(hipEventCreateWithFlags(&b->ev_md5, hipEventDisableTiming));
        const double t0 = now_ms();
        b->streams.resize(n);
        for (size_t i = 0; i < n; i++) {
            if (!streams[i].data && streams[i].len) return E_INVALID_ARGUMENT;
            plan_stream(b->streams[i], streams[i].data, streams[i].len);
        }
        const double t1 = now_ms();
        b->timings.plan_ms = t1 - t0;
        for (size_t i = 0; i < n; i++) {
            StreamState& s = b->streams[i];
            if (s.host_err || s.no_frames) continue;
            int ci = -1;
            for (size_t k = 0; k < b->classes.size(); k++)
                if (b->classes[k]->kind == s.kind && b->classes[k]->nch == s.nch) ci = (int)k;
            if (ci < 0) {
                b->classes.emplace_back(new Class());
                b->classes.back()->kind = s.kind;
                b->classes.back()->nch = s.nch;
                ci = (int)b->classes.size() - 1;
            }
            s.cls = ci;
            b->classes[ci]->members.push_back((uint32_t)i);
        }
        for (auto& C : b->classes) alloc_class(b.get(), *C, streams);
        if (flags & ZFLAC_FLAG_DEVICE_MD5) plan_md5_pipeline(b.get());
        b->timings.upload_ms = now_ms() - t1;
        for (auto& s : b->streams) {
            if (s.host_err) s.err = s.host_err;
            if (s.no_frames) {
                s.err = 0;
                s.info = zflac_info{};
                s.info.sample_kind = (uint8_t)s.kind;
            }
        }
    } catch (const DeviceError&) {
        return E_DEVICE;
    } catch (const std::bad_alloc&) {
        return E_OUT_OF_MEMORY;
    } catch (const std::exception&) {
        return E_DEVICE;
    }
    *out = b.release();
    return E_OK;
}

}
```

### zflac_amd/csrc/scan.hip

```cpp
#include "device_common.h"
#include "launch.h"

#ifndef ZFLAC_SCAN_AUX
#define ZFLAC_SCAN_AUX 0
#endif

namespace zflac {

__device__ inline uint32_t ff_mask(uint32_t d) { return ((d & 0x7F7F7F7Fu) + 0x01010101u) & d & 0x80808080u; }

template <typename Fn>
__device__ inline void scan_window_v(const uint4 v, const uint8_t* in, uint64_t ws, uint64_t lo, uint64_t hi, Fn&& fn) {
    const uint32_t d[4] = {v.x, v.y, v.z, v.w};
#pragma unroll
    for (int k = 0; k < 4; k++) {
        uint32_t m = ff_mask(d[k]);
        while (m) {
            const int bit = __ffs(m) - 1;
            m &= m - 1;
            const int b = 4 * k + (bit >> 3);
            uint32_t nxt;
            if (b < 15) nxt = (d[(b + 1) >> 2] >> (8 * ((b + 1) & 3))) & 0xFF;
            else nxt = in[ws + 16];
            const uint64_t p = ws + b;
            if ((nxt & 0xFE) == 0xF8 && p >= lo && p < hi) fn(p);
        }
    }
}
template <typename Fn>
__device__ inline void scan_window(const uint8_t* in, uint64_t ws, uint64_t lo, uint64_t hi, Fn&& fn) {
    scan_window_v(*reinterpret_cast<const uint4*>(in + ws), in, ws, lo, hi, fn);
}

__device__ __forceinline__ uint32_t sync_mask(uint32_t d, uint32_t dn) {
    const uint32_t nxt = __builtin_amdgcn_alignbyte(dn, d, 1);
    const uint32_t y = (nxt & 0xFEFEFEFEu) ^ 0xF8F8F8F8u;
    const uint32_t zero = ~(((y & 0x7F7F7F7Fu) + 0x7F7F7F7Fu) | y | 0x7F7F7F7Fu);
    return ff_mask(d) & zero;
}

__device__ __forceinline__ uint32_t sync_any(uint32_t d, uint32_t dn) {
    const uint32_t nxt = __builtin_amdgcn_alignbyte(dn, d, 1);
    const uint32_t t = ~d | ((nxt & 0xFEFEFEFEu) ^ 0xF8F8F8F8u);
    return (t - 0x01010101u) & ~t & 0x80808080u;
}

__device__ __forceinline__ uint32_t lane_above(uint32_t v) {
    return (uint32_t)__builtin_amdgcn_update_dpp(0, (int)v, 0x130, 0xf, 0xf, true);
}

struct ScanLds {
    uint32_t cnt;
    unsigned long long units;
    uint64_t pos[CHUNK_CAP];
    uint32_t u[CHUNK_CAP];
};


__device__ __forceinline__ void scan_chunk(const ScanArgs& a, uint32_t chunk, ScanLds& L) {
    const ChunkDesc ch = a.chunks[chunk];
    const uint64_t abase = ch.begin & ~(uint64_t)15;
    constexpr int R = SCAN_BYTES_PER_THREAD / 16;
    const __amdgpu_buffer_rsrc_t rs = __builtin_amdgcn_make_buffer_rsrc(
        const_cast<uint8_t*>(a.in) + abase, (short)0, (int)(ch.end - abase), 0x00020000);
    uint4 v[R];
#pragma unroll
    for (int r = 0; r < R; r++)
        v[r] = __builtin_bit_cast(uint4, __builtin_amdgcn_raw_buffer_load_b128(rs, threadIdx.x * 16u,
                                                                                 r * SCAN_THREADS * 16, ZFLAC_SCAN_AUX));
    const StreamDesc S = a.streams[ch.stream];
    if (threadIdx.x == 0) {
        L.cnt = 0;
        L.units = 0;
    }
    __syncthreads();
    const uint64_t lane_ws = abase + (uint64_t)threadIdx.x * 16;
#pragma unroll
    for (int r = 0; r < R; r++) {
        const uint64_t ws = lane_ws + (uint64_t)r * SCAN_THREADS * 16;
        const uint32_t n0 = lane_above(v[r].x);
        const bool nx_mem = (threadIdx.x & 63u) == 63u || ws + 16 >= ch.end;
        const bool maybe = ((sync_any(v[r].x, v[r].y) | sync_any(v[r].y, v[r].z) | sync_any(v[r].z, v[r].w) |
                             sync_any(v[r].w, n0)) != 0 ||
                            (nx_mem && (v[r].w >> 24) == 0xFFu)) &&
                           ws < ch.end;
        if (__builtin_amdgcn_ballot_w64(maybe) == 0) continue;
#if defined(ZFLAC_SCAN_ABL) && ZFLAC_SCAN_ABL == 2
        atomicAdd(&L.cnt, 1u);
        continue;
#endif
        const uint4 vn = make_uint4(n0, lane_above(v[r].y), lane_above(v[r].z), lane_above(v[r].w));
        if (ws >= ch.end) continue;
        const uint32_t c0 = sync_mask(v[r].x, v[r].y), c1 = sync_mask(v[r].y, v[r].z),
                       c2 = sync_mask(v[r].z, v[r].w);
        uint32_t c3 = sync_mask(v[r].w, n0);
        if (nx_mem && (v[r].w >> 24) == 0xFFu)
            c3 = (c3 & 0x00808080u) | ((a.in[ws + 16] & 0xFEu) == 0xF8u ? 0x80000000u : 0u);
        if ((c0 | c1 | c2 | c3) == 0 || ws >= ch.end) continue;
#if defined(ZFLAC_SCAN_ABL) && ZFLAC_SCAN_ABL == 1
        atomicAdd(&L.cnt, (uint32_t)__builtin_popcount(c0 | c1 | c2 | c3));
        continue;
#endif
        uint32_t cand = (c0 * 0x00204081u) >> 28 & 15u;
        cand |= ((c1 * 0x00204081u) >> 28 & 15u) << 4;
        cand |= ((c2 * 0x00204081u) >> 28 & 15u) << 8;
        cand |= ((c3 * 0x00204081u) >> 28 & 15u) << 12;
        const uint4 nx = nx_mem ? *reinterpret_cast<const uint4*>(a.in + ws + 16) : vn;
        while (cand) {
            const uint32_t b = (uint32_t)__ffs(cand) - 1u;
            cand &= cand - 1u;
            const uint64_t p = ws + b;
            if (p < ch.begin || p >= ch.end) continue;
            const bool s8 = (b & 8u) != 0, s4 = (b & 4u) != 0;
            const uint32_t x0 = s8 ? v[r].z : v[r].x, x1 = s8 ? v[r].w : v[r].y, x2 = s8 ? nx.x : v[r].z,
                           x3 = s8 ? nx.y : v[r].w, x4 = s8 ? nx.z : nx.x, x5 = s8 ? nx.w : nx.y;
            const uint32_t y0 = s4 ? x1 : x0, y1 = s4 ? x2 : x1, y2 = s4 ? x3 : x2, y3 = s4 ? x4 : x3,
                           y4 = s4 ? x5 : x4;
            const uint32_t sb = b & 3u;
            const uint32_t h0 = __builtin_amdgcn_alignbyte(y1, y0, sb), h1 = __builtin_amdgcn_alignbyte(y2, y1, sb),
                           h2 = __builtin_amdgcn_alignbyte(y3, y2, sb), h3 = __builtin_amdgcn_alignbyte(y4, y3, sb);
            const FrameHdr h = parse_frame_header_t<2>(
                [h0, h1, h2, h3](uint32_t i) -> uint32_t {
                    const uint32_t sel = (i & 7u) | 0x0C0C0C00u;
                    return (i & 8u) ? __builtin_amdgcn_perm(h3, h2, sel) : __builtin_amdgcn_perm(h1, h0, sel);
                },
                S.in_end - p, S.si_rate, nullptr);
            if (!candidate_ok(h, S)) continue;
            const uint32_t slot = atomicAdd(&L.cnt, 1u);
            const uint32_t units = h.bs * S.nch;
            atomicAdd(&L.units, (unsigned long long)units);
            if (slot < CHUNK_CAP) {
                L.pos[slot] = p;
                L.u[slot] = units;
            }
        }
    }
    __syncthreads();
    if (threadIdx.x == 0) {
        const uint32_t n = L.cnt;
        const uint32_t m = n < CHUNK_CAP ? n : CHUNK_CAP;
        for (uint32_t i = 1; i < m; i++) {
            uint64_t p = L.pos[i];
            uint32_t u = L.u[i];
            int j = (int)i - 1;
            while (j >= 0 && L.pos[j] > p) {
                L.pos[j + 1] = L.pos[j];
                L.u[j + 1] = L.u[j];
                j--;
            }
            L.pos[j + 1] = p;
            L.u[j + 1] = u;
        }
    }
    __syncthreads();
}

__device__ __forceinline__ void zero_run_words(const ScanArgs& a, uint32_t chunk) {
    for (uint32_t i = chunk * SCAN_THREADS + threadIdx.x; i < a.n_status; i += a.n_chunks * SCAN_THREADS)
        a.status[i] = 0;
    if (chunk == 0 && threadIdx.x < 4) a.misc[threadIdx.x] = 0;
}

__global__ __launch_bounds__(SCAN_THREADS) void k_scan(ScanArgs a) {
    const uint32_t chunk = blockIdx.x;
    if (chunk >= a.n_chunks) return;
    zero_run_words(a, chunk);
    __shared__ ScanLds L;
    scan_chunk(a, chunk, L);
    if (threadIdx.x == 0) {
        a.chunk_cnt[chunk] = L.cnt;
        a.chunk_units[chunk] = L.units;
    }
    const uint32_t m = L.cnt < CHUNK_CAP ? L.cnt : CHUNK_CAP;
    if (threadIdx.x < m) {
        a.chunk_slots[(uint64_t)chunk * CHUNK_CAP + threadIdx.x] = L.pos[threadIdx.x];
        a.chunk_slot_units[(uint64_t)chunk * CHUNK_CAP + threadIdx.x] = L.u[threadIdx.x];
    }
}

template <typename T>
__device__ __forceinline__ T wave_incl_sum(T v) {
    const uint32_t ln = threadIdx.x & 63u;
#pragma unroll
    for (int d = 1; d < 64; d <<= 1) {
        const T y = __shfl_up(v, d, 64);
        if (ln >= (uint32_t)d) v += y;
    }
    return v;
}

constexpr int SCANK_THREADS = 1024;
constexpr int SCANK_WAVES = SCANK_THREADS / 64;
constexpr int SCANK_T = 4;

__global__ __launch_bounds__(SCANK_THREADS) void k_scan_chunks(const uint32_t* cnt, const unsigned long long* units,
                                                               uint32_t n, uint32_t* off,
                                                               unsigned long long* uoff, uint32_t* n_frames) {
    __shared__ uint32_t s_c[SCANK_WAVES];
    __shared__ unsigned long long s_u[SCANK_WAVES];
    const uint32_t t = threadIdx.x, wv = t >> 6;
    uint32_t carry_c = 0;
    unsigned long long carry_u = 0;
    for (uint32_t tb = 0; tb < n; tb += SCANK_THREADS * SCANK_T) {
        const uint32_t i0 = tb + t * SCANK_T;
        uint32_t c[SCANK_T];
        unsigned long long u[SCANK_T];
        uint32_t sc = 0;
        unsigned long long su = 0;
#pragma unroll
        for (int i = 0; i < SCANK_T; i++) {
            const bool in = i0 + i < n;
            c[i] = in ? cnt[i0 + i] : 0u;
            u[i] = in ? units[i0 + i] : 0ull;
            sc += c[i];
            su += u[i];
        }
        const uint32_t ic = wave_incl_sum(sc);
        const unsigned long long iu = wave_incl_sum(su);
        if ((t & 63u) == 63u) {
            s_c[wv] = ic;
            s_u[wv] = iu;
        }
        __syncthreads();
        uint32_t rc = carry_c + ic - sc;
        unsigned long long ru = carry_u + iu - su;
        uint32_t tc = 0;
        unsigned long long tu = 0;
#pragma unroll
        for (uint32_t w = 0; w < (uint32_t)SCANK_WAVES; w++) {
            if (w < wv) {
                rc += s_c[w];
                ru += s_u[w];
            }
            tc += s_c[w];
            tu += s_u[w];
        }
#pragma unroll
        for (int i = 0; i < SCANK_T; i++) {
            if (i0 + i < n) {
                off[i0 + i] = rc;
                uoff[i0 + i] = ru;
            }
            rc += c[i];
            ru += u[i];
        }
        carry_c += tc;
        carry_u += tu;
        __syncthreads();
    }
    if (t == 0) {
        off[n] = carry_c;
        uoff[n] = carry_u;
        *n_frames = carry_c;
    }
}

constexpr int COMPACT_CHUNKS = SCAN_THREADS / 64;

__device__ void compact_rescan_at(const uint8_t* in, const StreamDesc* streams, const ChunkDesc* chunks, uint32_t chunk,
                                  uint32_t off, unsigned long long urel, uint32_t cap, uint64_t* c_pos,
                                  uint32_t* c_stream, uint64_t* c_out, uint32_t* overflow) {
    const ChunkDesc ch = chunks[chunk];
    const StreamDesc S = streams[ch.stream];
    auto parse = [&](uint64_t, uint64_t p) -> FrameHdr { return parse_frame_header(in + p, S.in_end - p, S.si_rate); };
    __shared__ uint32_t s_c[SCAN_THREADS];
    __shared__ unsigned long long s_u[SCAN_THREADS];
    __shared__ uint32_t s_base_c;
    __shared__ unsigned long long s_base_u;
    __syncthreads();
    if (threadIdx.x == 0) {
        s_base_c = 0;
        s_base_u = 0;
    }
    __syncthreads();
    const uint64_t abase = ch.begin & ~(uint64_t)15;
    for (int r = 0; r < SCAN_BYTES_PER_THREAD / 16; r++) {
        const uint64_t ws = abase + ((uint64_t)r * SCAN_THREADS + threadIdx.x) * 16;
        uint32_t c = 0;
        unsigned long long u = 0;
        if (ws < ch.end) {
            scan_window(in, ws, ch.begin, ch.end, [&](uint64_t p) {
                const FrameHdr h = parse(ws, p);
                if (!candidate_ok(h, S)) return;
                c++;
                u += h.bs * S.nch;
            });
        }
        s_c[threadIdx.x] = c;
        s_u[threadIdx.x] = u;
        __syncthreads();
        for (uint32_t d = 1; d < SCAN_THREADS; d <<= 1) {
            uint32_t vc = 0;
            unsigned long long vu = 0;
            if (threadIdx.x >= d) {
                vc = s_c[threadIdx.x - d];
                vu = s_u[threadIdx.x - d];
            }
            __syncthreads();
            s_c[threadIdx.x] += vc;
            s_u[threadIdx.x] += vu;
            __syncthreads();
        }
        uint32_t rc = s_base_c + s_c[threadIdx.x] - c;
        unsigned long long ru = s_base_u + s_u[threadIdx.x] - u;
        if (ws < ch.end && c) {
            scan_window(in, ws, ch.begin, ch.end, [&](uint64_t p) {
                const FrameHdr h = parse(ws, p);
                if (!candidate_ok(h, S)) return;
                const uint32_t idx = off + rc;
                if (idx < cap) {
                    c_pos[idx] = p;
                    c_stream[idx] = ch.stream;
                    c_out[idx] = S.out_base + (urel + ru);
                } else if (overflow) {
                    atomicOr(overflow, 1u);
                }
                rc++;
                ru += h.bs * S.nch;
            });
        }
        __syncthreads();
        if (threadIdx.x == SCAN_THREADS - 1) {
            s_base_c += s_c[threadIdx.x];
            s_base_u += s_u[threadIdx.x];
        }
        __syncthreads();
    }
}

__global__ __launch_bounds__(SCAN_THREADS) void k_compact(CompactArgs a) {
    const uint32_t c0 = blockIdx.x * COMPACT_CHUNKS;
    const uint32_t chunk = c0 + (threadIdx.x >> 6), ln = threadIdx.x & 63u;
    if (chunk < a.n_chunks) {
        const uint32_t n = a.chunk_cnt[chunk];
        if (n <= CHUNK_CAP) {
            const uint32_t stream = a.chunks[chunk].stream;
            const StreamDesc& S = a.streams[stream];
            const unsigned long long base = S.out_base + (a.chunk_uoff[chunk] - a.chunk_uoff[S.first_chunk]);
            const uint32_t u = ln < n ? a.chunk_slot_units[(uint64_t)chunk * CHUNK_CAP + ln] : 0u;
            const uint32_t pre = wave_incl_sum(u) - u;
            if (ln < n) {
                const uint32_t idx = a.chunk_off[chunk] + ln;
                if (idx < a.cap) {
                    a.c_pos[idx] = a.chunk_slots[(uint64_t)chunk * CHUNK_CAP + ln];
                    a.c_stream[idx] = stream;
                    a.c_out[idx] = base + pre;
                } else {
                    atomicOr(a.overflow, 1u);
                }
            }
        }
    }
#pragma unroll 1
    for (uint32_t j = 0; j < (uint32_t)COMPACT_CHUNKS; j++) {
        const uint32_t cj = c0 + j;
        if (cj < a.n_chunks && a.chunk_cnt[cj] > CHUNK_CAP) {
            const StreamDesc& S = a.streams[a.chunks[cj].stream];
            compact_rescan_at(a.in, a.streams, a.chunks, cj, a.chunk_off[cj],
                              a.chunk_uoff[cj] - a.chunk_uoff[S.first_chunk], a.cap, a.c_pos, a.c_stream, a.c_out,
                              a.overflow);
        }
    }
}

__global__ void k_verify(VerifyArgs a) {
    const uint32_t t = blockIdx.x * blockDim.x + threadIdx.x;
    uint32_t nframes = *a.n_frames;
    if (nframes > a.cap) nframes = a.cap;
    if (t < a.n_streams) {
        const StreamDesc S = a.streams[t];
        const uint32_t f0 = a.chunk_off[S.first_chunk], f1 = a.chunk_off[S.end_chunk];
        if (f1 <= f0 || f1 > nframes || (!S.valid_total && !a.units) || a.c_pos[f0] != S.in_begin)
            atomicOr(&a.status[t], 1u);
    }
    if (t >= nframes) return;
    const uint32_t s = a.c_stream[t];
    const StreamDesc S = a.streams[s];
    const uint32_t f1 = min(a.chunk_off[S.end_chunk], nframes);
    const uint64_t rel = a.c_out[t] - S.out_base;
    if (S.valid_total && rel >= S.total) return;
    bool bad = a.c_err[t] != 0;
    const uint32_t info = a.c_info[t];
    const uint32_t bs = (info & 0xFFFF) + 1;
    const uint32_t code = (info >> 16) & 15, dcode = (info >> 20) & 7;
    if ((uint32_t)channels_count(code) != S.nch || dcode != S.dcode || a.c_rate[t] != S.rate_hz) bad = true;
    const uint64_t units = (uint64_t)bs * S.nch;
    if (bs == 1 && rel + S.nch < S.total) bad = true;
    const uint64_t end_rel = rel + units;
    if (end_rel > S.out_cap) bad = true;
    if (S.valid_total) {
        if (end_rel > S.total) bad = true;
        if (end_rel < S.total && (t + 1 >= f1 || a.c_pos[t + 1] != a.c_end[t])) bad = true;
    } else {
        const bool last = a.c_end[t] + 4 > S.in_end;
        if (!last && (t + 1 >= f1 || a.c_pos[t + 1] != a.c_end[t])) bad = true;
        if (last && t + 1 < f1) bad = true;
        if (last && a.units) a.units[s] = end_rel;
    }
    if (bad) atomicOr(&a.status[s], 1u);
}

__global__ __launch_bounds__(SCAN_THREADS) void k_sync_list(SyncListArgs a) {
    const uint64_t abase = a.lo & ~(uint64_t)15;
    const uint64_t nwin = (a.hi - abase + 15) / 16;
    for (uint64_t w = (uint64_t)blockIdx.x * SCAN_THREADS + threadIdx.x; w < nwin;
         w += (uint64_t)gridDim.x * SCAN_THREADS) {
        scan_window(a.in, abase + w * 16, a.lo, a.hi, [&](uint64_t p) {
            const FrameHdr h = parse_frame_header(a.in + p, a.in_end - p, a.si_rate);
            if (h.err || h.crc_eof || channels_count(h.chan_code) != a.nch || h.dcode != a.dcode ||
                h.rate != a.rate_hz)
                return;
            const uint32_t slot = atomicAdd(a.count, 1u);
            if (slot < a.cap) a.pos[slot] = p;
        });
    }
}

hipError_t launch_scan(const ScanArgs& a, hipStream_t st) {
    if (a.n_chunks == 0) return hipSuccess;
    hipLaunchKernelGGL(k_scan, dim3(a.n_chunks), dim3(SCAN_THREADS), 0, st, a);
    return hipGetLastError();
}
hipError_t launch_scan_chunks(const uint32_t* cnt, const unsigned long long* units, uint32_t n, uint32_t* off,
                              unsigned long long* uoff, uint32_t* n_frames, hipStream_t st) {
    hipLaunchKernelGGL(k_scan_chunks, dim3(1), dim3(SCANK_THREADS), 0, st, cnt, units, n, off, uoff, n_frames);
    return hipGetLastError();
}
hipError_t launch_compact(const CompactArgs& a, hipStream_t st) {
    if (a.n_chunks == 0) return hipSuccess;
    hipLaunchKernelGGL(k_compact, dim3((a.n_chunks + COMPACT_CHUNKS - 1) / COMPACT_CHUNKS), dim3(SCAN_THREADS), 0, st,
                       a);
    return hipGetLastError();
}
hipError_t launch_sync_list(const SyncListArgs& a, hipStream_t st) {
    if (a.hi <= a.lo) return hipSuccess;
    const uint64_t windows = (a.hi - (a.lo & ~(uint64_t)15) + 15) / 16;
    uint64_t blocks = (windows + SCAN_THREADS - 1) / SCAN_THREADS;
    if (blocks > 4096) blocks = 4096;
    hipLaunchKernelGGL(k_sync_list, dim3((uint32_t)blocks), dim3(SCAN_THREADS), 0, st, a);
    return hipGetLastError();
}
hipError_t launch_verify(const VerifyArgs& a, uint32_t max_items, hipStream_t st) {
    uint32_t n = max_items > a.n_streams ? max_items : a.n_streams;
    uint32_t blocks = (n + 255) / 256;
    if (blocks == 0) blocks = 1;
    hipLaunchKernelGGL(k_verify, dim3(blocks), dim3(256), 0, st, a);
    return hipGetLastError();
}

}
```

### zflac_amd/csrc/stream_plan.cpp

```cpp
#include "stream_plan.h"

#include <cstring>

namespace zflac {

namespace {
struct ByteReader {
    const uint8_t* d;
    size_t n;
    size_t pos = 0;
    bool get(size_t k, uint64_t& v) {
        if (n - pos < k) return false;
        v = 0;
        for (size_t i = 0; i < k; i++) v = (v << 8) | d[pos + i];
        pos += k;
        return true;
    }
};
}

int parse_metadata(const uint8_t* d, size_t n, StreamInfoH& si, size_t& frames_begin) {
    ByteReader r{d, n};
    uint64_t v;
    if (!r.get(4, v)) return E_END_OF_STREAM;
    if (v != 0x664C6143) return E_INVALID_SIGNATURE;
    bool have = false;
    for (;;) {
        uint64_t h;
        if (!r.get(4, h)) return E_END_OF_STREAM;
        const unsigned info = (unsigned)(h >> 24) & 0x7F;
        const bool last = (h >> 31) & 1;
        const uint64_t length = h & 0xFFFFFF;
        if (info == 0) {
            if (r.n - r.pos < 34) return E_END_OF_STREAM;
            const uint8_t* p = d + r.pos;
            si.min_block = (uint16_t)((p[0] << 8) | p[1]);
            si.max_block = (uint16_t)((p[2] << 8) | p[3]);
            si.sample_rate = ((uint32_t)p[10] << 12) | ((uint32_t)p[11] << 4) | (p[12] >> 4);
            si.channels = ((p[12] >> 1) & 7) + 1;
            si.bps = (((p[12] & 1) << 4) | (p[13] >> 4)) + 1;
            si.total = ((uint64_t)(p[13] & 15) << 32) | ((uint64_t)p[14] << 24) | ((uint64_t)p[15] << 16) |
                       ((uint64_t)p[16] << 8) | p[17];
            std::memcpy(si.md5, p + 18, 16);
            r.pos += 34;
            have = true;
        } else if (info >= 1 && info <= 6) {
            if (r.n - r.pos < length) return E_END_OF_STREAM;
            r.pos += length;
        } else {
            return E_INVALID_METADATA_HEADER;
        }
        if (last) break;
    }
    if (!have) return E_MISSING_STREAMINFO;
    frames_begin = r.pos;
    return E_OK;
}

int kind_of_bps(uint32_t bps) {
    const uint32_t aligned = (bps + 7) / 8 * 8;
    if (aligned == 8) return 0;
    if (aligned == 16) return 1;
    return 2;
}
int esz_of_kind(int kind) { return kind == 0 ? 1 : (kind == 1 ? 2 : 4); }
uint8_t justify_of(uint32_t bps) {
    if (bps >= 9 && bps <= 15) return (uint8_t)(16 - bps);
    if (bps >= 17 && bps <= 31) return (uint8_t)(32 - bps);
    return 0;
}

void plan_stream(StreamPlan& s, const uint8_t* d, size_t n) {
    s.len = n;
    s.host_err = parse_metadata(d, n, s.si, s.frames_begin);
    if (s.host_err) return;
    s.kind = kind_of_bps(s.si.bps);
    s.nch = (int)s.si.channels;
    const bool valid_total = s.si.total > 0;
    const uint64_t avail = n - s.frames_begin;
    if (avail < 4) {
        if (valid_total) s.host_err = E_END_OF_STREAM;
        else s.no_frames = true;
        return;
    }
    const uint8_t* p = d + s.frames_begin;
    s.first = parse_frame_header_t<0>([p](uint32_t i) -> uint32_t { return p[i]; }, avail, s.si.sample_rate, nullptr);
    if (s.first.err) { s.host_err = s.first.err; return; }
    if (depth_bits(s.first.dcode, (int)s.si.bps) < 0) { s.host_err = E_OUT_OF_DOMAIN; return; }
    if (channels_count(s.first.chan_code) != s.nch) { s.host_err = E_INCONSISTENT_PARAMETERS; return; }
}

}
```

### zflac_amd/csrc/stream_plan.h

```cpp
#pragma once
#include <cstddef>
#include <cstdint>

#include "common.h"
#include "frame_header.h"

namespace zflac {

struct StreamInfoH {
    uint16_t min_block = 0, max_block = 0;
    uint32_t sample_rate = 0;
    uint32_t channels = 0;
    uint32_t bps = 0;
    uint64_t total = 0;
    uint8_t md5[16] = {};
};

struct StreamPlan {
    int host_err = 0;
    StreamInfoH si;
    size_t len = 0;
    size_t frames_begin = 0;
    int kind = 1;
    int nch = 0;
    FrameHdr first = {};
    bool no_frames = false;
};

int parse_metadata(const uint8_t* d, size_t n, StreamInfoH& si, size_t& frames_begin);

int kind_of_bps(uint32_t bps);
int esz_of_kind(int kind);
uint8_t justify_of(uint32_t bps);

void plan_stream(StreamPlan& s, const uint8_t* d, size_t n);

}
```

Before: 767,700 Msamples/s.

## Add hop front-end that jumps between fixed-size frames instead of full scanning

Adds a 'hop' frame-location kernel for fixed-blocksize streams. It predicts each next frame start from the previous frame's length and probes small windows around that guess, checking the sync pattern, the header CRC and the coded frame number. This replaces the full byte scan, chunk prefix-sum and compaction passes with one launch when a class has enough streams (default at least 768) with few frames each. If any hop fails, the class falls back to the scan path and is re-run, which costs extra host synchronisation and planning work.

Measured after the change: 911,200 Msamples/s, median of 6. 1.19x the previous value.

```diff
diff --git a/include/zflac_hip.h b/include/zflac_hip.h
--- a/include/zflac_hip.h
+++ b/include/zflac_hip.h
@@ -95,6 +95,9 @@
 #define ZFLAC_BUCKET_12 64u
 #define ZFLAC_BUCKET_ALL 127u
 int zflac_hip_batch_decode_buckets(zflac_batch *b, uint32_t *used, uint32_t *planned);
+#define ZFLAC_FRONT_SCAN 1
+#define ZFLAC_FRONT_HOP 2
+int zflac_hip_batch_front(zflac_batch *b, int *planned, int *used);
 size_t zflac_hip_batch_size(zflac_batch *b);
 void zflac_hip_batch_destroy(zflac_batch *b);
 
@@ -138,6 +141,8 @@
 #define ZFLAC_FLAG_CHECK_CRC16 8
 #define ZFLAC_FLAG_WALK_LANE 16
 #define ZFLAC_FLAG_WALK_WAVE 32
+#define ZFLAC_FLAG_FRONT_SCAN 64
+#define ZFLAC_FLAG_FRONT_HOP 128
 
 const char *zflac_hip_error_name(int code);
 int zflac_hip_device_count(void);
diff --git a/zflac_amd/_lib.py b/zflac_amd/_lib.py
--- a/zflac_amd/_lib.py
+++ b/zflac_amd/_lib.py
@@ -70,6 +70,7 @@
                                                        ctypes.POINTER(ctypes.c_uint64)]),
     "zflac_hip_batch_decode_buckets": (ctypes.c_int, [_P, ctypes.POINTER(ctypes.c_uint32),
                                                       ctypes.POINTER(ctypes.c_uint32)]),
+    "zflac_hip_batch_front": (ctypes.c_int, [_P, ctypes.POINTER(ctypes.c_int), ctypes.POINTER(ctypes.c_int)]),
     "zflac_hip_batch_size": (ctypes.c_size_t, [_P]),
     "zflac_hip_batch_destroy": (None, [_P]),
     "zflac_hip_error_name": (ctypes.c_char_p, [ctypes.c_int]),
@@ -84,6 +85,8 @@
 FLAG_CHECK_CRC16 = 8
 FLAG_WALK_LANE = 16
 FLAG_WALK_WAVE = 32
+FLAG_FRONT_SCAN = 64
+FLAG_FRONT_HOP = 128
 EXPORT_F32 = 0
 EXPORT_F16 = 1
 EXPORT_BF16 = 2
@@ -98,6 +101,8 @@
 BUCKET_MIX_32 = 32
 BUCKET_12 = 64
 BUCKET_ALL = 127
+FRONT_SCAN = 1
+FRONT_HOP = 2
 
 _lib = None
 
diff --git a/zflac_amd/api.py b/zflac_amd/api.py
--- a/zflac_amd/api.py
+++ b/zflac_amd/api.py
@@ -96,7 +96,8 @@
 class Batch:
 
     def __init__(self, streams, device: int = 0, timing: bool = False, force_slow: bool = False,
-                 device_md5: bool = False, check_crc16: bool = False, walk: str | None = None):
+                 device_md5: bool = False, check_crc16: bool = False, walk: str | None = None,
+                 front: str | None = None):
         self._L = _lib.load()
         self.device = device
         self._bufs = [bytes(s) for s in streams]
@@ -109,7 +110,8 @@
             arr[i].len = len(b)
         flags = ((_lib.FLAG_TIMING if timing else 0) | (_lib.FLAG_FORCE_SLOW if force_slow else 0)
                  | (_lib.FLAG_DEVICE_MD5 if device_md5 else 0) | (_lib.FLAG_CHECK_CRC16 if check_crc16 else 0)
-                 | {None: 0, "lane": _lib.FLAG_WALK_LANE, "wave": _lib.FLAG_WALK_WAVE}[walk])
+                 | {None: 0, "lane": _lib.FLAG_WALK_LANE, "wave": _lib.FLAG_WALK_WAVE}[walk]
+                 | {None: 0, "auto": 0, "scan": _lib.FLAG_FRONT_SCAN, "hop": _lib.FLAG_FRONT_HOP}[front])
         self._h = ctypes.c_void_p()
         rc = self._L.zflac_hip_batch_create(arr, len(self._bufs), device, flags, ctypes.byref(self._h))
         self._keep = None
@@ -165,6 +167,11 @@
         errors.check(self._L.zflac_hip_batch_decode_buckets(self._h, ctypes.byref(used), ctypes.byref(planned)),
                      "batch_decode_buckets")
         return used.value, planned.value
+
+    def front(self):
+        planned, used = ctypes.c_int(), ctypes.c_int()
+        errors.check(self._L.zflac_hip_batch_front(self._h, ctypes.byref(planned), ctypes.byref(used)), "batch_front")
+        return planned.value, used.value
 
     def device_samples(self, i: int) -> int:
         return self._L.zflac_hip_batch_device_samples(self._h, i) or 0
diff --git a/zflac_amd/build.py b/zflac_amd/build.py
--- a/zflac_amd/build.py
+++ b/zflac_amd/build.py
@@ -11,7 +11,7 @@
 LIB = os.path.join(HERE, "libzflac_hip.so")
 SOURCES = [os.path.join(CSRC, f"decode_k{k}_{lay}{mix}.hip") for k in (1, 2, 0) for lay in ("stereo", "mono", "multi")
            for mix in ("", "_mix")]
-SOURCES += [os.path.join(CSRC, n) for n in ("scan.hip", "md5.hip", "crc16.hip", "walk_wave.hip", "export.hip",
+SOURCES += [os.path.join(CSRC, n) for n in ("scan.hip", "hop.hip", "md5.hip", "crc16.hip", "walk_wave.hip", "export.hip",
                                             "resample.hip", "stream_plan.cpp", "resample_plan.cpp", "pipeline.cpp",
                                             "seq_planner.cpp", "md5_host.cpp", "abi.cpp")]
 HEADERS = [os.path.join(CSRC, n) for n in ("common.h", "frame_header.h", "device_common.h", "launch.h", "stream_plan.h",
diff --git a/zflac_amd/csrc/abi.cpp b/zflac_amd/csrc/abi.cpp
--- a/zflac_amd/csrc/abi.cpp
+++ b/zflac_amd/csrc/abi.cpp
@@ -502,6 +502,16 @@
     return E_OK;
 }
 
+static_assert(ZFLAC_FRONT_SCAN == FRONT_SCAN && ZFLAC_FRONT_HOP == FRONT_HOP,
+              "ZFLAC_FRONT_* (zflac_hip.h) and Front (stream_plan.h) disagree");
+
+int zflac_hip_batch_front(zflac_batch* b, int* planned, int* used) {
+    if (!b || !planned || !used || !b->ran || b->submitted) return E_INVALID_ARGUMENT;
+    *planned = b->front_planned;
+    *used = b->front_used;
+    return E_OK;
+}
+
 int zflac_hip_batch_export_ms(zflac_batch* b, double* ms) {
     if (!b || !ms || b->export_ms < 0) return E_INVALID_ARGUMENT;
     *ms = b->export_ms;
@@ -535,6 +545,10 @@
                 Class& C = *b->classes[0];
                 if (what == 4) {
                     enqueue_class(b, C, false, false);
+                    continue;
+                }
+                if (what >= 8 && C.front == FRONT_HOP) {
+                    ck(launch_hop(hop_args(C), b->rs));
                     continue;
                 }
                 if (what >= 8) {
diff --git a/zflac_amd/csrc/batch.h b/zflac_amd/csrc/batch.h
--- a/zflac_amd/csrc/batch.h
+++ b/zflac_amd/csrc/batch.h
@@ -76,6 +76,12 @@
     uint32_t grid_frames = 0;
     uint32_t full_mask = 0;
     bool redone = false;
+    Front front = FRONT_SCAN;
+    Front front_run = FRONT_SCAN, front_used = FRONT_SCAN;
+    std::vector<HopDesc> hop;
+    DevBuf<HopDesc> d_hop;
+    uint32_t hop_frames = 0;
+    uint32_t hop_epoch = 0;
     DevBuf<uint8_t> in;
     DevBuf<uint8_t> out;
     DevBuf<StreamDesc> d_desc;
@@ -156,6 +162,7 @@
 DecodeArgs decode_args(Class& C);
 ScanArgs scan_args(Class& C);
 CompactArgs compact_args(Class& C);
+HopArgs hop_args(Class& C);
 hipError_t launch_decode(int kind, const DecodeArgs& a, uint32_t max_frames, hipStream_t st,
                          hipEvent_t mid = nullptr, hipStream_t front = nullptr, hipEvent_t join = nullptr,
                          uint64_t est_frames = 0, int flags = 0);
@@ -206,5 +213,6 @@
     std::vector<std::unique_ptr<zflac::ResampleTable>> rs_tables;
     uint64_t rs_built = 0;
     uint32_t buckets_used = 0, buckets_planned = 0;
+    int front_planned = 0, front_used = 0;
     ~zflac_batch();
 };
diff --git a/zflac_amd/csrc/common.h b/zflac_amd/csrc/common.h
--- a/zflac_amd/csrc/common.h
+++ b/zflac_amd/csrc/common.h
@@ -88,6 +88,39 @@
     uint32_t* misc;
 };
 
+struct HopDesc {
+    uint32_t n_frames;
+    uint32_t f0;
+    uint32_t units;
+    uint32_t guess;
+};
+static_assert(sizeof(HopDesc) == 16, "HopDesc is the 16-byte record host and kernel share");
+
+#ifndef ZFLAC_HOP_MAX_FRAMES
+#define ZFLAC_HOP_MAX_FRAMES 64
+#endif
+#ifndef ZFLAC_HOP_MIN_STREAMS
+#define ZFLAC_HOP_MIN_STREAMS 768
+#endif
+constexpr uint32_t HOP_MAX_FRAMES = ZFLAC_HOP_MAX_FRAMES;
+constexpr uint32_t HOP_MIN_STREAMS = ZFLAC_HOP_MIN_STREAMS;
+
+struct HopArgs {
+    const uint8_t* in;
+    const StreamDesc* streams;
+    const HopDesc* hop;
+    uint32_t n_streams;
+    uint32_t total_frames;
+    uint32_t cap;
+    uint32_t epoch;
+    uint64_t* c_pos;
+    uint32_t* c_stream;
+    uint64_t* c_out;
+    uint32_t* chunk_off;
+    uint32_t* status;
+    uint32_t* misc;
+};
+
 struct CompactArgs {
     const uint8_t* in;
     const StreamDesc* streams;
diff --git a/zflac_amd/csrc/device_common.h b/zflac_amd/csrc/device_common.h
--- a/zflac_amd/csrc/device_common.h
+++ b/zflac_amd/csrc/device_common.h
@@ -21,6 +21,21 @@
     return parse_frame_header_t<0>([p](uint32_t i) -> uint32_t { return p[i]; }, avail, si_rate, nullptr);
 }
 
+__device__ inline uint32_t ff_mask(uint32_t d) { return ((d & 0x7F7F7F7Fu) + 0x01010101u) & d & 0x80808080u; }
+
+__device__ __forceinline__ uint32_t sync_mask(uint32_t d, uint32_t dn) {
+    const uint32_t nxt = __builtin_amdgcn_alignbyte(dn, d, 1);
+    const uint32_t y = (nxt & 0xFEFEFEFEu) ^ 0xF8F8F8F8u;
+    const uint32_t zero = ~(((y & 0x7F7F7F7Fu) + 0x7F7F7F7Fu) | y | 0x7F7F7F7Fu);
+    return ff_mask(d) & zero;
+}
+
+__device__ __forceinline__ uint32_t sync_any(uint32_t d, uint32_t dn) {
+    const uint32_t nxt = __builtin_amdgcn_alignbyte(dn, d, 1);
+    const uint32_t t = ~d | ((nxt & 0xFEFEFEFEu) ^ 0xF8F8F8F8u);
+    return (t - 0x01010101u) & ~t & 0x80808080u;
+}
+
 __device__ __forceinline__ bool candidate_ok(const FrameHdr& h, const StreamDesc& S) {
     return h.err == 0 && !h.crc_eof && h.crc_ok && h.zero_bit == 0 && h.byte1 == S.byte1 &&
            channels_count(h.chan_code) == S.nch && h.dcode == S.dcode && h.rate == S.rate_hz;
diff --git a/zflac_amd/csrc/frame_header.h b/zflac_amd/csrc/frame_header.h
--- a/zflac_amd/csrc/frame_header.h
+++ b/zflac_amd/csrc/frame_header.h
@@ -188,4 +188,27 @@
     return h;
 }
 
-}
+template <typename At>
+ZFLAC_HDI bool coded_number_value(At&& at, uint64_t avail, uint64_t& value) {
+    value = 0;
+    if (avail <= 4) return false;
+    const uint32_t first = at(4);
+    uint32_t ones = 0;
+    ZFLAC_UNROLL
+    for (int k = 0; k < 8; k++)
+        if (ones == (uint32_t)k && (first & (0x80u >> k))) ones++;
+    if (first == 0xFF || ones == 1) return false;
+    if (ones == 0) {
+        value = first;
+        return true;
+    }
+    if (avail < (uint64_t)4 + ones) return false;
+    uint64_t v = first & (0x7Fu >> ones);
+    ZFLAC_UNROLL
+    for (uint32_t k = 1; k < 7; k++)
+        if (k < ones) v = (v << 6) | (at(4 + k) & 0x3Fu);
+    value = v;
+    return true;
+}
+
+}
diff --git a/zflac_amd/csrc/hop.hip b/zflac_amd/csrc/hop.hip
--- /dev/null
+++ b/zflac_amd/csrc/hop.hip
@@ -0,0 +1,170 @@
+#include "device_common.h"
+#include "launch.h"
+
+namespace zflac {
+
+constexpr int HOP_LANES = 16;
+constexpr int HOP_LANE_BYTES = 64;
+constexpr int HOP_WINDOW = HOP_LANES * HOP_LANE_BYTES;
+constexpr int HOP_PROBES = 16;
+constexpr int HOP_THREADS = 64;
+
+__device__ __forceinline__ uint32_t hop_group_min(uint32_t v) {
+#pragma unroll
+    for (int m = HOP_LANES / 2; m; m >>= 1) v = min(v, (uint32_t)__shfl_xor((int)v, m, HOP_LANES));
+    return v;
+}
+
+struct HopHit {
+    uint32_t pos, higher;
+};
+
+__device__ __forceinline__ HopHit hop_probe_lane(const __amdgpu_buffer_rsrc_t rs, const StreamDesc& S, uint64_t abase,
+                                                 int64_t off, uint32_t lo, uint32_t end, uint64_t want,
+                                                 uint64_t want_units) {
+    HopHit hit{~0u, 0u};
+    if (off < 0 || off >= (int64_t)end) return hit;
+    uint32_t d[20];
+#pragma unroll
+    for (int j = 0; j < 5; j++) {
+        const uint4 v = __builtin_bit_cast(uint4, __builtin_amdgcn_raw_buffer_load_b128(rs, (uint32_t)off, j * 16, 0));
+        d[4 * j] = v.x;
+        d[4 * j + 1] = v.y;
+        d[4 * j + 2] = v.z;
+        d[4 * j + 3] = v.w;
+    }
+    uint32_t any = 0;
+#pragma unroll
+    for (int i = 0; i < 16; i++) any |= sync_any(d[i], d[i + 1]);
+    if (!any) return hit;
+    uint64_t cand = 0;
+#pragma unroll
+    for (int i = 0; i < 16; i++)
+        cand |= (uint64_t)((sync_mask(d[i], d[i + 1]) * 0x00204081u) >> 28 & 15u) << (4 * i);
+    while (cand) {
+        const uint32_t b = (uint32_t)__ffsll((unsigned long long)cand) - 1u;
+        cand &= cand - 1;
+        const uint64_t rel = (uint64_t)off + b;
+        if (rel < lo || rel >= end) continue;
+        const uint32_t dw = b >> 2, sb = b & 3u;
+        uint32_t w0 = 0, w1 = 0, w2 = 0, w3 = 0, w4 = 0;
+#pragma unroll
+        for (int i = 0; i < 16; i++) {
+            const bool here = dw == (uint32_t)i;
+            w0 = here ? d[i] : w0;
+            w1 = here ? d[i + 1] : w1;
+            w2 = here ? d[i + 2] : w2;
+            w3 = here ? d[i + 3] : w3;
+            w4 = here ? d[i + 4] : w4;
+        }
+        const uint32_t h0 = __builtin_amdgcn_alignbyte(w1, w0, sb), h1 = __builtin_amdgcn_alignbyte(w2, w1, sb),
+                       h2 = __builtin_amdgcn_alignbyte(w3, w2, sb), h3 = __builtin_amdgcn_alignbyte(w4, w3, sb);
+        auto at = [h0, h1, h2, h3](uint32_t i) -> uint32_t {
+            const uint32_t sel = (i & 7u) | 0x0C0C0C00u;
+            return (i & 8u) ? __builtin_amdgcn_perm(h3, h2, sel) : __builtin_amdgcn_perm(h1, h0, sel);
+        };
+        const uint64_t avail = S.in_end - (abase + rel);
+        const FrameHdr h = parse_frame_header_t<2>(at, avail, S.si_rate, nullptr);
+        if (!candidate_ok(h, S)) continue;
+        uint64_t num;
+        if (!coded_number_value(at, avail, num)) continue;
+        if (num == want) {
+            if (hit.pos == ~0u && (uint64_t)h.bs * S.nch == want_units) hit.pos = (uint32_t)rel;
+        } else if (num > want) {
+            hit.higher = 1;
+        }
+    }
+    return hit;
+}
+
+__global__ __launch_bounds__(HOP_THREADS) void k_hop(HopArgs a) {
+    if (blockIdx.x == 0 && threadIdx.x == 0) {
+        a.misc[0] = a.total_frames;
+        a.misc[1] = 0;
+        a.misc[2] = 0;
+    }
+    const uint32_t s = (blockIdx.x * HOP_THREADS + threadIdx.x) / HOP_LANES;
+    if (s >= a.n_streams) return;
+    const uint32_t ln = threadIdx.x & (HOP_LANES - 1);
+    const StreamDesc S = a.streams[s];
+    const HopDesc H = a.hop[s];
+    const uint64_t abase = S.in_begin & ~(uint64_t)15;
+    const uint32_t end = (uint32_t)(S.in_end - abase);
+    const uint32_t begin = (uint32_t)(S.in_begin - abase);
+    const __amdgpu_buffer_rsrc_t rs = __builtin_amdgcn_make_buffer_rsrc(
+        const_cast<uint8_t*>(a.in) + abase, (short)0, (int)((end + 15u) & ~15u), 0x00020000);
+    auto put = [&](uint32_t i, uint64_t pos) {
+        if (ln == 0 && H.f0 + i < a.cap) {
+            a.c_pos[H.f0 + i] = pos;
+            a.c_stream[H.f0 + i] = s;
+            a.c_out[H.f0 + i] = S.out_base + (uint64_t)i * H.units;
+        }
+    };
+    uint32_t cur;
+    {
+        const HopHit hit = hop_probe_lane(rs, S, abase, (int64_t)ln * HOP_LANE_BYTES, begin, end, 0,
+                                          H.n_frames > 1 ? (uint64_t)H.units : S.total);
+        cur = hop_group_min(hit.pos);
+    }
+    bool failed = cur != begin;
+    uint32_t done = 0;
+    if (!failed) {
+        put(0, S.in_begin);
+        done = 1;
+        uint32_t guess = H.guess;
+        for (uint32_t f = 0; f + 1 < H.n_frames; f++) {
+            const int64_t lo_ws = (int64_t)((cur + 1u) & ~15u);
+            int64_t ws0 = ((int64_t)cur + guess - HOP_WINDOW / 2) & ~(int64_t)15;
+            if (ws0 < lo_ws) ws0 = lo_ws;
+            const uint64_t want_units = f + 2 < H.n_frames ? (uint64_t)H.units : S.total - (uint64_t)(f + 1) * H.units;
+            int fwd = 0, back = -1, dir = 0;
+            uint32_t found = ~0u;
+#pragma unroll 1
+            for (int pr = 0; pr < HOP_PROBES; pr++) {
+                const bool back_ok = ws0 + (int64_t)(back + 1) * HOP_WINDOW > lo_ws;
+                const bool fwd_ok = ws0 + (int64_t)fwd * HOP_WINDOW < (int64_t)end;
+                bool go_back = dir < 0 || (dir == 0 && (pr & 1));
+                if (go_back && !back_ok) {
+                    if (dir < 0) break;
+                    go_back = false;
+                }
+                if (!go_back && !fwd_ok) {
+                    if (dir > 0 || !back_ok) break;
+                    go_back = true;
+                }
+                const int k = go_back ? back-- : fwd++;
+                const int64_t ws = ws0 + (int64_t)k * HOP_WINDOW;
+                const HopHit hit = hop_probe_lane(rs, S, abase, ws + (int64_t)ln * HOP_LANE_BYTES, cur + 1u, end,
+                                                  (uint64_t)f + 1, want_units);
+                found = hop_group_min(hit.pos);
+                if (found != ~0u) break;
+                if (hop_group_min(hit.higher ? 0u : 1u) == 0u) dir = -1;
+                else if (!back_ok) dir = 1;
+            }
+            if (found == ~0u) {
+                failed = true;
+                break;
+            }
+            guess = found - cur;
+            cur = found;
+            put(f + 1, abase + cur);
+            done = f + 2;
+        }
+    }
+    for (uint32_t i = done; i < H.n_frames; i++) put(i, S.in_end);
+    if (ln == 0) {
+        a.chunk_off[S.first_chunk] = H.f0;
+        a.chunk_off[S.end_chunk] = H.f0 + H.n_frames;
+        a.status[s] = failed ? 2u : 0u;
+        if (failed) a.misc[3] = a.epoch;
+    }
+}
+
+hipError_t launch_hop(const HopArgs& a, hipStream_t st) {
+    if (a.n_streams == 0) return hipSuccess;
+    const uint32_t per = HOP_THREADS / HOP_LANES;
+    hipLaunchKernelGGL(k_hop, dim3((a.n_streams + per - 1) / per), dim3(HOP_THREADS), 0, st, a);
+    return hipGetLastError();
+}
+
+}
diff --git a/zflac_amd/csrc/launch.h b/zflac_amd/csrc/launch.h
--- a/zflac_amd/csrc/launch.h
+++ b/zflac_amd/csrc/launch.h
@@ -13,6 +13,8 @@
 hipError_t launch_compact(const CompactArgs& a, hipStream_t st);
 hipError_t launch_sync_list(const SyncListArgs& a, hipStream_t st);
 hipError_t launch_verify(const VerifyArgs& a, uint32_t max_items, hipStream_t st);
+
+hipError_t launch_hop(const HopArgs& a, hipStream_t st);
 
 using DecodeLaunch = hipError_t(const DecodeArgs& a, uint32_t max_frames, hipStream_t st);
 DecodeLaunch launch_decode_k0_stereo, launch_decode_k0_mono, launch_decode_k0_multi;
diff --git a/zflac_amd/csrc/pipeline.cpp b/zflac_amd/csrc/pipeline.cpp
--- a/zflac_amd/csrc/pipeline.cpp
+++ b/zflac_amd/csrc/pipeline.cpp
@@ -100,6 +100,8 @@
         cands[C.chunks[k].stream] += cnt[k];
     }
 }
+
+void plan_front(zflac_batch* b, Class& C);
 
 void alloc_class(zflac_batch* b, Class& C, const zflac_stream* src) {
     C.full_mask = plan_buckets(b, C, src);
@@ -170,6 +172,7 @@
     C.chunk_off.alloc(nc + 1);
     C.chunk_uoff.alloc(nc + 1);
     C.misc.alloc(4 + C.members.size());
+    ck(hipMemset(C.misc.p, 0, (4 + C.members.size()) * sizeof(uint32_t)));
     C.status = C.misc.p + 4;
     C.dummy.alloc(DUMMY_BYTES + PROBE_BYTES);
     if (C.any_unknown) {
@@ -237,6 +240,35 @@
     C.cap = (uint32_t)std::min<uint64_t>(est_frames + C.chunks.size() * 2 + 1024, 0x7FFFFFFFull);
     C.est_frames = est_frames;
     C.grid_frames = (uint32_t)std::min<uint64_t>(grid_frames + grid_frames / 64 + 64, C.cap);
+    plan_front(b, C);
+}
+
+FrontMode front_mode(int flags) {
+    const int f = flags & (ZFLAC_FLAG_FRONT_SCAN | ZFLAC_FLAG_FRONT_HOP);
+    if (f == ZFLAC_FLAG_FRONT_SCAN) return FRONT_FORCE_SCAN;
+    if (f == ZFLAC_FLAG_FRONT_HOP) return FRONT_FORCE_HOP;
+    if (f) return FRONT_AUTO;
+    const char* e = std::getenv("ZFLAC_FRONT");
+    return !e ? FRONT_AUTO : (e[0] == 's' ? FRONT_FORCE_SCAN : (e[0] == 'h' ? FRONT_FORCE_HOP : FRONT_AUTO));
+}
+
+void plan_front(zflac_batch* b, Class& C) {
+    HopLimits lim;
+    if (const char* e = std::getenv("ZFLAC_HOP_MAX_FRAMES")) lim.max_frames = (uint32_t)std::strtoul(e, nullptr, 10);
+    if (const char* e = std::getenv("ZFLAC_HOP_MIN_STREAMS")) lim.min_streams = (uint32_t)std::strtoul(e, nullptr, 10);
+    std::vector<const StreamPlan*> plans(C.members.size());
+    for (size_t m = 0; m < C.members.size(); m++) plans[m] = &b->streams[C.members[m]];
+    C.hop.resize(C.members.size());
+    uint64_t total = 0;
+    C.front = plan_hop(plans.data(), plans.size(), front_mode(b->flags), lim, C.hop.data(), &total);
+    if (C.front == FRONT_HOP && total > C.cap) C.front = FRONT_SCAN;
+    if (C.front != FRONT_HOP) {
+        C.hop.clear();
+        return;
+    }
+    C.hop_frames = (uint32_t)total;
+    C.d_hop.alloc(C.hop.size());
+    ck(hipMemcpy(C.d_hop.p, C.hop.data(), C.hop.size() * sizeof(HopDesc), hipMemcpyHostToDevice));
 }
 
 void alloc_candidates(Class& C) {
@@ -287,6 +319,26 @@
     a.c_stream = C.c_stream.p;
     a.c_out = C.c_out.p;
     a.overflow = C.misc.p + 1;
+    return a;
+}
+
+HopArgs hop_args(Class& C) {
+    HopArgs a;
+    std::memset(&a, 0, sizeof(a));
+    a.in = C.in.p;
+    a.streams = C.d_desc.p;
+    a.hop = C.d_hop.p;
+    a.n_streams = (uint32_t)C.members.size();
+    a.total_frames = C.hop_frames;
+    a.cap = C.cap;
+    if (++C.hop_epoch == 0) C.hop_epoch = 1;
+    a.epoch = C.hop_epoch;
+    a.c_pos = C.c_pos.p;
+    a.c_stream = C.c_stream.p;
+    a.c_out = C.c_out.p;
+    a.chunk_off = C.chunk_off.p;
+    a.status = C.status;
+    a.misc = C.misc.p;
     return a;
 }
 
@@ -397,9 +449,14 @@
     if (nch == 0)
         ck(hipMemsetAsync(C.misc.p, 0, (4 + C.members.size()) * sizeof(uint32_t), st));
     if (timing_first) ck(hipEventRecord(b->ev[0], st));
-    ck(launch_scan(scan_args(C), st));
-    if (nch) ck(launch_scan_chunks(C.chunk_cnt.p, C.chunk_units.p, nch, C.chunk_off.p, C.chunk_uoff.p, C.misc.p, st));
-    ck(launch_compact(compact_args(C), st));
+    C.front_run = C.front;
+    if (C.front == FRONT_HOP) {
+        ck(launch_hop(hop_args(C), st));
+    } else {
+        ck(launch_scan(scan_args(C), st));
+        if (nch) ck(launch_scan_chunks(C.chunk_cnt.p, C.chunk_units.p, nch, C.chunk_off.p, C.chunk_uoff.p, C.misc.p, st));
+        ck(launch_compact(compact_args(C), st));
+    }
     if (timing_last) ck(hipEventRecord(b->ev[1], st));
     DecodeArgs da = decode_args(C);
     da.bucket_used = C.misc.p + 2;
@@ -477,9 +534,19 @@
         ck(hipEventSynchronize(b->ev_md5));
     }
     uint32_t rest_launches = 0, sequential = 0, used = 0, planned = 0;
+    b->front_planned = b->front_used = 0;
     for (size_t ci = 0; ci < b->classes.size(); ci++) {
         Class& C = *b->classes[ci];
         planned |= C.full_mask;
+        b->front_planned |= C.front_run;
+        C.front_used = C.front_run;
+        if (C.front_run == FRONT_HOP && C.h_misc[3] == C.hop_epoch) {
+            C.front = C.front_used = FRONT_SCAN;
+            C.redone = true;
+            enqueue_class(b, C, false, false);
+            ck(hipStreamSynchronize(b->stream));
+        }
+        b->front_used |= C.front_used;
         for (int attempt = 0; attempt < 3; attempt++) {
             if (!C.h_misc[1] && C.h_misc[0] <= C.cap) break;
             C.cap = std::max<uint32_t>(C.h_misc[0] + 1024, C.cap * 2);
diff --git a/zflac_amd/csrc/scan.hip b/zflac_amd/csrc/scan.hip
--- a/zflac_amd/csrc/scan.hip
+++ b/zflac_amd/csrc/scan.hip
@@ -7,7 +7,6 @@
 
 namespace zflac {
 
-__device__ inline uint32_t ff_mask(uint32_t d) { return ((d & 0x7F7F7F7Fu) + 0x01010101u) & d & 0x80808080u; }
 
 template <typename Fn>
 __device__ inline void scan_window_v(const uint4 v, const uint8_t* in, uint64_t ws, uint64_t lo, uint64_t hi, Fn&& fn) {
@@ -30,19 +29,6 @@
 template <typename Fn>
 __device__ inline void scan_window(const uint8_t* in, uint64_t ws, uint64_t lo, uint64_t hi, Fn&& fn) {
     scan_window_v(*reinterpret_cast<const uint4*>(in + ws), in, ws, lo, hi, fn);
-}
-
-__device__ __forceinline__ uint32_t sync_mask(uint32_t d, uint32_t dn) {
-    const uint32_t nxt = __builtin_amdgcn_alignbyte(dn, d, 1);
-    const uint32_t y = (nxt & 0xFEFEFEFEu) ^ 0xF8F8F8F8u;
-    const uint32_t zero = ~(((y & 0x7F7F7F7Fu) + 0x7F7F7F7Fu) | y | 0x7F7F7F7Fu);
-    return ff_mask(d) & zero;
-}
-
-__device__ __forceinline__ uint32_t sync_any(uint32_t d, uint32_t dn) {
-    const uint32_t nxt = __builtin_amdgcn_alignbyte(dn, d, 1);
-    const uint32_t t = ~d | ((nxt & 0xFEFEFEFEu) ^ 0xF8F8F8F8u);
-    return (t - 0x01010101u) & ~t & 0x80808080u;
 }
 
 __device__ __forceinline__ uint32_t lane_above(uint32_t v) {
diff --git a/zflac_amd/csrc/stream_plan.cpp b/zflac_amd/csrc/stream_plan.cpp
--- a/zflac_amd/csrc/stream_plan.cpp
+++ b/zflac_amd/csrc/stream_plan.cpp
@@ -90,4 +90,39 @@
     if (channels_count(s.first.chan_code) != s.nch) { s.host_err = E_INCONSISTENT_PARAMETERS; return; }
 }
 
+uint32_t hop_frames(const StreamPlan& s) {
+    const uint64_t bs = s.si.min_block;
+    return bs ? (uint32_t)((s.si.total + bs - 1) / bs) : 0;
 }
+
+bool hop_stream_ok(const StreamPlan& s, uint32_t max_frames) {
+    if (s.host_err || s.no_frames || s.si.total == 0) return false;
+    if (s.si.min_block != s.si.max_block || s.si.min_block < 16 || s.first.byte1 != 0xF8) return false;
+    if ((s.si.total + s.si.min_block - 1) / s.si.min_block > max_frames) return false;
+    return s.len - s.frames_begin < (1ull << 31);
+}
+
+Front plan_hop(const StreamPlan* const* streams, size_t n, FrontMode mode, const HopLimits& lim, HopDesc* out,
+               uint64_t* total_frames) {
+    if (total_frames) *total_frames = 0;
+    if (mode == FRONT_FORCE_SCAN || n == 0) return FRONT_SCAN;
+    if (mode == FRONT_AUTO && n < lim.min_streams) return FRONT_SCAN;
+    uint64_t f0 = 0;
+    for (size_t i = 0; i < n; i++) {
+        const StreamPlan& s = *streams[i];
+        if (!hop_stream_ok(s, lim.max_frames)) return FRONT_SCAN;
+        const uint32_t nf = hop_frames(s);
+        if (f0 + nf > 0x7FFFFFFFull) return FRONT_SCAN;
+        if (out) {
+            out[i].n_frames = nf;
+            out[i].f0 = (uint32_t)f0;
+            out[i].units = (uint32_t)s.si.min_block * (uint32_t)s.nch;
+            out[i].guess = (uint32_t)((s.len - s.frames_begin) / nf);
+        }
+        f0 += nf;
+    }
+    if (total_frames) *total_frames = f0;
+    return FRONT_HOP;
+}
+
+}
diff --git a/zflac_amd/csrc/stream_plan.h b/zflac_amd/csrc/stream_plan.h
--- a/zflac_amd/csrc/stream_plan.h
+++ b/zflac_amd/csrc/stream_plan.h
@@ -35,4 +35,17 @@
 
 void plan_stream(StreamPlan& s, const uint8_t* d, size_t n);
 
+enum Front : int { FRONT_SCAN = 1, FRONT_HOP = 2 };
+enum FrontMode : int { FRONT_AUTO = 0, FRONT_FORCE_SCAN = 1, FRONT_FORCE_HOP = 2 };
+
+struct HopLimits {
+    uint32_t max_frames = HOP_MAX_FRAMES;
+    uint32_t min_streams = HOP_MIN_STREAMS;
+};
+
+bool hop_stream_ok(const StreamPlan& s, uint32_t max_frames);
+uint32_t hop_frames(const StreamPlan& s);
+Front plan_hop(const StreamPlan* const* streams, size_t n, FrontMode mode, const HopLimits& lim, HopDesc* out,
+               uint64_t* total_frames);
+
 }
```
